# bcgsc/ntSynt

Hardware: AMD Instinct MI355X
Metric: minimizer-sketch Gbases/s (sketch with common Bloom filter, inputs resident in HBM) (higher is better)
Workload: dtype u64

## Files before the change

include/ntsynt_hip.h:

```cpp
#ifndef NTSYNT_HIP_H
#define NTSYNT_HIP_H

#include <stdint.h>

#ifdef __cplusplus
extern "C" {
#endif

#define NTS_OK 0
#define NTS_EINVAL (-22)
#define NTS_ENOMEM (-12)
#define NTS_EHIP (-5)
#define NTS_ERANGE (-34)
#define NTS_EFORMAT (-74)
#define NTS_ECOMM (-70)

typedef struct nts_ctx nts_ctx;
typedef struct nts_genome nts_genome;
typedef struct nts_bf nts_bf;
typedef struct nts_mx nts_mx;
typedef struct nts_hset nts_hset;
typedef struct nts_hcount nts_hcount;
typedef struct nts_comm nts_comm;

// ... 44 lines not shown
#define NTS_SYNTH_NRUN 4u
typedef struct
{
  uint64_t dst, len, src;
  uint32_t flags, reserved;
} nts_synth_piece;
int nts_genome_synth_plan(nts_ctx* ctx, uint32_t n_rec, const uint64_t* rec_len, uint32_t n_pieces, const nts_synth_piece* pieces,
                          uint64_t seed_ancestor, uint64_t seed_genome, double substitution_rate, nts_genome** out);
#define NTS_SYNTH_TANDEM 8u
typedef struct
{
  uint32_t sine_cell_log2, sine_len, sine_prob_256, sine_families;
  uint32_t line_cell_log2, line_len, line_min_len, line_prob_256, line_families;
  uint32_t div_min_1024, div_max_1024;
  uint32_t sat_unit, sat_div_1024;
} nts_synth_repeats;
int nts_genome_synth_plan_ex(nts_ctx* ctx, uint32_t n_rec, const uint64_t* rec_len, uint32_t n_pieces, const nts_synth_piece* pieces,
                             uint64_t seed_ancestor, uint64_t seed_genome, double substitution_rate, const nts_synth_repeats* rep,
                             nts_genome** out);
int nts_genome_download(nts_ctx* ctx, const nts_genome* g, uint64_t offset, uint64_t len, uint8_t* ascii);
uint64_t nts_genome_bases(const nts_genome* g);
int nts_genome_valid_kmers(nts_ctx* ctx, const nts_genome* g, uint32_t k, uint64_t* n_valid);

int nts_bf_create(nts_ctx* ctx, uint64_t bytes, nts_bf** out);
void nts_bf_free(nts_ctx* ctx, nts_bf* bf);
uint64_t nts_bf_bytes(const nts_bf* bf);
void* nts_bf_device_ptr(nts_bf* bf);
int nts_bf_clear(nts_ctx* ctx, nts_bf* bf);
int nts_bf_insert_and(nts_ctx* ctx, nts_bf* acc, const nts_genome* g, uint32_t k);
int nts_bf_insert(nts_ctx* ctx, nts_bf* bf, const nts_genome* g, uint32_t k);
int nts_bf_build_mode(nts_ctx* ctx, int mode);
int nts_bf_cascade(nts_ctx* ctx, const nts_bf* prev, nts_bf* next, const nts_genome* g, uint32_t k);
int nts_bf_insert_repeats(nts_ctx* ctx, nts_bf* genome_bf, nts_bf* repeat_bf, const nts_genome* g, uint32_t k);
int nts_bf_and(nts_ctx* ctx, nts_bf* acc, const nts_bf* other);
int nts_bf_popcount(nts_ctx* ctx, const nts_bf* bf, uint64_t* bits_set);
int nts_bf_download(nts_ctx* ctx, const nts_bf* bf, uint8_t* host, uint64_t bytes);
int nts_bf_upload(nts_ctx* ctx, nts_bf* bf, const uint8_t* host, uint64_t bytes);
int nts_bf_save(nts_ctx* ctx, const nts_bf* bf, const char* path, const void* header, uint64_t header_bytes, uint32_t n_threads);
int nts_bench_random_probe(nts_ctx* ctx, const nts_bf* bf, uint64_t n_probes, uint32_t repeats, double* avg_ms, uint64_t* hits);
int nts_bench_valu(nts_ctx* ctx, int kind, uint32_t waves_per_simd, uint32_t iters, double* wall_ms, double* cycles_per_instr,
                   double* instr_per_wave);
int nts_mod_indices(nts_ctx* ctx, uint64_t bits, int form, const uint64_t* h, uint64_t n, uint64_t* out);
int nts_bf_wrap(nts_ctx* ctx, void* device_ptr, uint64_t bytes, nts_bf** out);
int nts_and_raw(nts_ctx* ctx, void* acc_dev, const void* other_dev, uint64_t bytes);

int nts_comm_unique_id(uint8_t* id128);
int nts_comm_init(nts_ctx* ctx, const uint8_t* id128, int world, int rank, nts_comm** out);
int nts_comm_wrap(nts_ctx* ctx, void* rccl_comm, nts_comm** out);
void nts_comm_destroy(nts_comm* comm);
int nts_comm_world(const nts_comm* comm);
int nts_comm_rank(const nts_comm* comm);
void* nts_comm_handle(const nts_comm* comm);
const char* nts_comm_library(void);
int nts_bf_create_sharded(nts_ctx* ctx, uint64_t bytes, int world, nts_bf** out);
int nts_bf_fill_ones(nts_ctx* ctx, nts_bf* bf);
int nts_bf_allreduce_and(nts_ctx* ctx, nts_bf* bf, nts_comm* comm);
int nts_bf_allreduce_groups(nts_ctx* ctx, nts_bf* bf, nts_comm* comm, const int32_t* group_of, uint32_t n_groups);
int nts_comm_last_sparse(const nts_ctx* ctx);
int nts_comm_last_exchange2(const nts_ctx* ctx, uint64_t* packed_bytes, uint64_t* unpacked_bytes, uint64_t* sent_bytes);
int nts_bf_allreduce_parts(nts_ctx* ctx, nts_bf* const* bfs, uint32_t n_local, nts_comm* comm, uint32_t n_slots, const int32_t* slot_group,
                           uint32_t n_groups);
int nts_mx_allgather(nts_ctx* ctx, nts_comm* comm, uint32_t n_local, const nts_mx* const* local, const uint32_t* local_ids,
                     uint32_t n_total, nts_mx** out);
int nts_mx_allgather_ex(nts_ctx* ctx, nts_comm* comm, uint32_t n_local, const nts_mx* const* local, const uint32_t* local_ids,
                        uint32_t n_total, uint32_t slots_per_rank, nts_mx** out);

int nts_sketch(nts_ctx* ctx,
               const nts_genome* g,
               uint32_t k,
               uint32_t w,
               const nts_bf* filter_or_null,
               const nts_interval* mask,
               uint64_t n_mask,
               nts_mx** out);

int nts_sketch_ex(nts_ctx* ctx, const nts_genome* g, uint32_t k, uint32_t w, const nts_bf* filter, const nts_bf* filter_out,
                  const nts_interval* mask, uint64_t n_mask, nts_mx** out);
int nts_sketch_mode(nts_ctx* ctx, int mode, uint32_t prune_c);
int nts_sketch_summary(nts_ctx* ctx, int mode, uint32_t* last_shift);
int nts_sketch_select(nts_ctx* ctx, int impl);
int nts_sketch_tiers(nts_ctx* ctx, int mode, double x0, int half_steps, uint64_t* last_probes, uint64_t* last_rounds, uint32_t* last_tiers);
int nts_sketch_stats(nts_ctx* ctx, uint64_t* candidates, uint64_t* uncovered_ranges, uint64_t* uncovered_kmers, uint32_t* prune_c_used);
int nts_path_stats(nts_ctx* ctx, uint64_t* sketch_many_listed, uint64_t* bf_direct_indices, uint32_t* bf_list_fallback);
int nts_bf_level_stats(nts_ctx* ctx, uint32_t* sparse_level, uint64_t* accepted_kmers);
uint64_t nts_mx_count(const nts_mx* mx);
void nts_mx_free(nts_ctx* ctx, nts_mx* mx);
int nts_mx_download(nts_ctx* ctx, const nts_mx* mx, uint64_t* h1, uint32_t* rec, uint64_t* pos);
int nts_mx_device_ptrs(const nts_mx* mx, void** h1, void** rec, void** pos);
int nts_mx_export(nts_ctx* ctx, const nts_mx* mx, void* h1_dev, void* rec_dev, void* pos_dev);
int nts_mx_export_async(nts_ctx* ctx, const nts_mx* mx, void* h1_dev, void* rec_dev, void* pos_dev);
int nts_mx_kmers(nts_ctx* ctx, const nts_genome* g, const nts_mx* mx, uint32_t k, uint8_t* host);
int nts_mx_split(nts_ctx* ctx, const nts_mx* mx, uint32_t n_parts, const uint32_t* rec_base, nts_mx** out);
int nts_mx_concat(nts_ctx* ctx, uint32_t n_parts, const nts_mx* const* parts, const uint32_t* rec_offset, nts_mx** out);
int nts_mx_screen(nts_ctx* ctx, const nts_genome* g, const nts_mx* mx, uint32_t k, const nts_bf* filter_out, nts_mx** out);
int nts_mx_upload(nts_ctx* ctx,
                  const uint64_t* h1,
                  const uint32_t* rec,
                  const uint64_t* pos,
                  uint64_t n,
                  nts_mx** out);

int nts_hash_all(nts_ctx* ctx, const nts_genome* g, uint32_t k, uint64_t** h0, uint64_t* n_out);

int nts_minhash(nts_ctx* ctx, const nts_genome* g, uint32_t k, uint32_t s, uint64_t* out, uint32_t* n_out);

int nts_minhash_intervals(nts_ctx* ctx, const nts_genome* g, uint32_t k, uint32_t s, const nts_interval* iv, uint64_t n_iv, uint64_t* out,
                          uint32_t* n_out, uint64_t* n_kmers);
int nts_minhash_intervals_stats(nts_ctx* ctx, uint32_t* passes, uint32_t* chunks, uint64_t* sweeps);
int nts_minhash_pairs(nts_ctx* ctx, uint32_t s, const uint64_t* sk, const uint32_t* n_sk, uint64_t n_sketches, const uint64_t* pair_a,
                      const uint64_t* pair_b, uint64_t n_pairs, uint32_t* shared, uint32_t* usize);

int nts_bf_count_intervals(nts_ctx* ctx, const nts_genome* g, uint32_t k, const nts_bf* bf, const nts_interval* iv, uint64_t n_iv,
                           uint64_t* n_kmers, uint64_t* n_hits);
int nts_genome_valid_bases(nts_ctx* ctx, const nts_genome* g, const nts_interval* iv, uint64_t n_iv, uint64_t* n_valid);

typedef struct
{
  uint64_t h0;
  uint32_t iv;
  uint32_t off;
} nts_sample;
typedef struct
{
  uint32_t list_a, iv_a, list_b, iv_b;
  uint32_t anchors, fwd, rev;
  uint32_t min_off_a, max_off_a, min_off_b, max_off_b;
} nts_iv_link;
int nts_bf_sample_intervals(nts_ctx* ctx, const nts_genome* g, uint32_t k, const nts_bf* bf, uint64_t rate, const nts_interval* iv,
                            uint64_t n_iv, uint64_t* n_sampled, nts_sample** out, uint64_t* n_out);
int nts_iv_links(nts_ctx* ctx, uint32_t n_lists, const nts_sample* const* lists, const uint64_t* n, uint32_t min_anchors, nts_iv_link** out,
                 uint64_t* n_out);

int nts_hset_build(nts_ctx* ctx, const uint64_t* h, uint64_t n, nts_hset** out);
void nts_hset_free(nts_ctx* ctx, nts_hset* set);
int nts_hset_contains(nts_ctx* ctx, const nts_hset* set, const uint64_t* h, uint64_t n, uint8_t* out);
int nts_hset_sample_intervals(nts_ctx* ctx, const nts_genome* g, uint32_t k, const nts_hset* set, uint64_t rate, const nts_interval* iv,
                              uint64_t n_iv, uint64_t* n_sampled, nts_sample** out, uint64_t* n_out);

int nts_hcount_create(nts_ctx* ctx, const nts_hset* set, nts_hcount** out);
int nts_hcount_clear(nts_ctx* ctx, nts_hcount* cnt);
void nts_hcount_free(nts_ctx* ctx, nts_hcount* cnt);
int nts_hcount_add(nts_ctx* ctx, const nts_hset* set, nts_hcount* cnt, const uint64_t* h, uint64_t n);
int nts_hcount_read(nts_ctx* ctx, const nts_hset* set, const nts_hcount* cnt, const uint64_t* h, uint64_t n, uint32_t* out);
int nts_hset_count_intervals(nts_ctx* ctx, const nts_genome* g, uint32_t k, const nts_hset* set, nts_hcount* cnt, uint64_t rate,
                             const nts_interval* iv, uint64_t n_iv, uint64_t* n_hits);

typedef struct
{
  uint32_t list_q, iv_q, rec_t;
  uint32_t hits, fwd, rev;
  uint32_t min_off_q, max_off_q, first_t, last_t;
} nts_iv_site;
int nts_hset_sample_intervals_capped(nts_ctx* ctx, const nts_genome* g, uint32_t k, const nts_hset* set, const nts_hcount* cnt, uint32_t cap,
                                     uint64_t rate, const nts_interval* iv, uint64_t n_iv, uint64_t* n_sampled, nts_sample** out, uint64_t* n_out);
int nts_iv_sites(nts_ctx* ctx, uint32_t n_lists, const nts_sample* const* lists, const uint64_t* n, const nts_sample* target, uint64_t n_target,
                 uint32_t step, uint32_t min_hits, nts_iv_site** out, uint64_t* n_out);

typedef struct
{
  uint32_t recurring, period, period_hits, first_off, last_off;
} nts_iv_period;
int nts_sample_intervals(nts_ctx* ctx, const nts_genome* g, uint32_t k, uint64_t rate, const nts_interval* iv, uint64_t n_iv, uint64_t* n_sampled,
                         nts_sample** out, uint64_t* n_out);
int nts_iv_periods(nts_ctx* ctx, const nts_sample* recs, uint64_t n, uint64_t n_iv, nts_iv_period* out);

typedef struct
// ... 137 lines not shown
```

ntsynt_amd/_lib.py:

```python
import ctypes
import os
import subprocess

_HERE = os.path.dirname(os.path.abspath(__file__))
LIB_PATH = os.path.join(_HERE, "libntsynt_hip.so")
EXP_LIB_PATH = os.path.join(_HERE, "libntsynt_hip_exp.so")

c_u8p = ctypes.POINTER(ctypes.c_uint8)
c_u32p = ctypes.POINTER(ctypes.c_uint32)
c_i64p = ctypes.POINTER(ctypes.c_int64)
c_u64p = ctypes.POINTER(ctypes.c_uint64)
c_vp = ctypes.c_void_p
u32, u64 = ctypes.c_uint32, ctypes.c_uint64


class Interval(ctypes.Structure):
    _fields_ = [("rec", u32), ("start", u64), ("end", u64)]


class Sample(ctypes.Structure):
    _fields_ = [("h0", u64), ("iv", u32), ("off", u32)]


class IvLink(ctypes.Structure):
# ... 45 lines not shown
class Blocks(ctypes.Structure):
    _fields_ = [("n_blocks", u64), ("first_vid", c_u32p), ("last_vid", c_u32p), ("n_mx", c_u32p), ("rec", c_u32p),
                ("first_pos", c_u64p), ("last_pos", c_u64p), ("ori", c_u8p), ("stats_paths", u64), ("stats_unoriented", u64),
                ("stats_indel_cuts", u64), ("stats_small", u64)]


SYMBOLS = [
    ("nts_init", ctypes.c_int, [ctypes.c_int, ctypes.POINTER(c_vp)]),
    ("nts_destroy", None, [c_vp]),
    ("nts_last_error", ctypes.c_char_p, [c_vp]),
    ("nts_sync", ctypes.c_int, [c_vp]),
    ("nts_stream", c_vp, [c_vp]),
    ("nts_profile", ctypes.c_int, [c_vp, ctypes.c_int]),
    ("nts_timing", ctypes.c_int, [c_vp, ctypes.c_char_p, ctypes.POINTER(ctypes.c_double), c_u64p]),
    ("nts_mem_stats", ctypes.c_int, [c_vp, c_u64p, c_u64p, c_u64p, c_u64p]),
    ("nts_mem_reset_peak", None, []),
    ("nts_bf_size_bytes", ctypes.c_int, [u64, ctypes.c_double, c_u64p, c_u64p]),
    ("nts_bf_size_bytes_ex", ctypes.c_int, [u64, ctypes.c_double, ctypes.c_int, c_u64p, c_u64p]),
    ("nts_genome_upload", ctypes.c_int, [c_vp, c_vp, u64, c_u64p, c_u64p, u32, ctypes.POINTER(c_vp)]),
    ("nts_genome_synth", ctypes.c_int, [c_vp, u64, u32, u64, u64, ctypes.c_double, ctypes.POINTER(c_vp)]),
    ("nts_genome_synth_plan", ctypes.c_int, [c_vp, u32, c_vp, u32, c_vp, u64, u64, ctypes.c_double, ctypes.POINTER(c_vp)]),
    ("nts_genome_synth_plan_ex", ctypes.c_int, [c_vp, u32, c_vp, u32, c_vp, u64, u64, ctypes.c_double, c_vp, ctypes.POINTER(c_vp)]),
    ("nts_genome_download", ctypes.c_int, [c_vp, c_vp, u64, u64, c_vp]),
    ("nts_genome_concat", ctypes.c_int, [c_vp, u32, c_vp, ctypes.POINTER(c_vp)]),
    ("nts_genome_slice", ctypes.c_int, [c_vp, c_vp, u32, u32, ctypes.POINTER(c_vp)]),
    ("nts_genome_free", None, [c_vp, c_vp]),
    ("nts_genome_bases", u64, [c_vp]),
    ("nts_genome_valid_kmers", ctypes.c_int, [c_vp, c_vp, u32, c_u64p]),
    ("nts_bf_create", ctypes.c_int, [c_vp, u64, ctypes.POINTER(c_vp)]),
    ("nts_bf_free", None, [c_vp, c_vp]),
    ("nts_bf_bytes", u64, [c_vp]),
    ("nts_bf_device_ptr", c_vp, [c_vp]),
    ("nts_bf_clear", ctypes.c_int, [c_vp, c_vp]),
    ("nts_bf_insert", ctypes.c_int, [c_vp, c_vp, c_vp, u32]),
    ("nts_bf_insert_and", ctypes.c_int, [c_vp, c_vp, c_vp, u32]),
    ("nts_bf_build_mode", ctypes.c_int, [c_vp, ctypes.c_int]),
    ("nts_bf_cascade", ctypes.c_int, [c_vp, c_vp, c_vp, c_vp, u32]),
    ("nts_bf_insert_repeats", ctypes.c_int, [c_vp, c_vp, c_vp, c_vp, u32]),
    ("nts_bf_and", ctypes.c_int, [c_vp, c_vp, c_vp]),
    ("nts_bf_popcount", ctypes.c_int, [c_vp, c_vp, c_u64p]),
    ("nts_bf_download", ctypes.c_int, [c_vp, c_vp, c_vp, u64]),
    ("nts_bf_upload", ctypes.c_int, [c_vp, c_vp, c_vp, u64]),
    ("nts_bf_save", ctypes.c_int, [c_vp, c_vp, ctypes.c_char_p, c_vp, u64, u32]),
    ("nts_bench_random_probe", ctypes.c_int, [c_vp, c_vp, u64, u32, ctypes.POINTER(ctypes.c_double), c_u64p]),
    ("nts_bench_valu", ctypes.c_int, [c_vp, ctypes.c_int, u32, u32, ctypes.POINTER(ctypes.c_double),
                                      ctypes.POINTER(ctypes.c_double), ctypes.POINTER(ctypes.c_double)]),
    ("nts_mod_indices", ctypes.c_int, [c_vp, u64, ctypes.c_int, c_vp, u64, c_vp]),
    ("nts_bf_wrap", ctypes.c_int, [c_vp, c_vp, u64, ctypes.POINTER(c_vp)]),
    ("nts_and_raw", ctypes.c_int, [c_vp, c_vp, c_vp, u64]),
    ("nts_comm_unique_id", ctypes.c_int, [c_vp]),
    ("nts_comm_init", ctypes.c_int, [c_vp, c_vp, ctypes.c_int, ctypes.c_int, ctypes.POINTER(c_vp)]),
    ("nts_comm_wrap", ctypes.c_int, [c_vp, c_vp, ctypes.POINTER(c_vp)]),
    ("nts_comm_destroy", None, [c_vp]),
    ("nts_comm_world", ctypes.c_int, [c_vp]),
    ("nts_comm_rank", ctypes.c_int, [c_vp]),
    ("nts_comm_handle", c_vp, [c_vp]),
    ("nts_comm_library", ctypes.c_char_p, []),
    ("nts_bf_create_sharded", ctypes.c_int, [c_vp, u64, ctypes.c_int, ctypes.POINTER(c_vp)]),
    ("nts_bf_fill_ones", ctypes.c_int, [c_vp, c_vp]),
    ("nts_bf_allreduce_and", ctypes.c_int, [c_vp, c_vp, c_vp]),
    ("nts_bf_allreduce_groups", ctypes.c_int, [c_vp, c_vp, c_vp, ctypes.POINTER(ctypes.c_int32), u32]),
    ("nts_comm_last_sparse", ctypes.c_int, [c_vp]),
    ("nts_comm_last_exchange2", ctypes.c_int, [c_vp, c_vp, c_vp, c_vp]),
    ("nts_mx_allgather", ctypes.c_int, [c_vp, c_vp, u32, ctypes.POINTER(c_vp), c_u32p, u32, ctypes.POINTER(c_vp)]),
    ("nts_alloc_stats", ctypes.c_int, [c_vp, c_vp]),
    ("nts_mem_trim", ctypes.c_uint64, []),
    ("nts_mem_cache_stats", ctypes.c_int, [c_vp, c_vp]),
    ("nts_mem_reserve", ctypes.c_int, [ctypes.c_int, ctypes.c_uint64, c_vp]),
    ("nts_mem_events", ctypes.c_int, [c_vp]),
    ("nts_mx_allgather_ex", ctypes.c_int, [c_vp, c_vp, u32, ctypes.POINTER(c_vp), c_u32p, u32, u32, ctypes.POINTER(c_vp)]),
    ("nts_bf_allreduce_parts", ctypes.c_int, [c_vp, ctypes.POINTER(c_vp), u32, c_vp, u32, ctypes.POINTER(ctypes.c_int32), u32]),
    ("nts_mx_export", ctypes.c_int, [c_vp, c_vp, c_vp, c_vp, c_vp]),
    ("nts_mx_export_async", ctypes.c_int, [c_vp, c_vp, c_vp, c_vp, c_vp]),
    ("nts_sketch", ctypes.c_int, [c_vp, c_vp, u32, u32, c_vp, ctypes.POINTER(Interval), u64,
                                  ctypes.POINTER(c_vp)]),
    ("nts_sketch_ex", ctypes.c_int, [c_vp, c_vp, u32, u32, c_vp, c_vp, ctypes.POINTER(Interval), u64,
                                     ctypes.POINTER(c_vp)]),
    ("nts_sketch_mode", ctypes.c_int, [c_vp, ctypes.c_int, u32]),
    ("nts_sketch_summary", ctypes.c_int, [c_vp, ctypes.c_int, c_u32p]),
    ("nts_sketch_select", ctypes.c_int, [c_vp, ctypes.c_int]),
    ("nts_sketch_tiers", ctypes.c_int, [c_vp, ctypes.c_int, ctypes.c_double, ctypes.c_int, ctypes.c_void_p, ctypes.c_void_p, ctypes.c_void_p]),
    ("nts_sketch_stats", ctypes.c_int, [c_vp, c_u64p, c_u64p, c_u64p, c_u32p]),
    ("nts_path_stats", ctypes.c_int, [c_vp, c_u64p, c_u64p, c_u32p]),
    ("nts_bf_level_stats", ctypes.c_int, [c_vp, c_u32p, c_u64p]),
    ("nts_mx_count", u64, [c_vp]),
    ("nts_mx_free", None, [c_vp, c_vp]),
    ("nts_mx_download", ctypes.c_int, [c_vp, c_vp, c_vp, c_vp, c_vp]),
    ("nts_mx_device_ptrs", ctypes.c_int, [c_vp, ctypes.POINTER(c_vp), ctypes.POINTER(c_vp),
                                          ctypes.POINTER(c_vp)]),
    ("nts_mx_split", ctypes.c_int, [c_vp, c_vp, u32, c_u32p, ctypes.POINTER(c_vp)]),
    ("nts_mx_concat", ctypes.c_int, [c_vp, u32, ctypes.POINTER(c_vp), c_u32p, ctypes.POINTER(c_vp)]),
    ("nts_mx_screen", ctypes.c_int, [c_vp, c_vp, c_vp, u32, c_vp, ctypes.POINTER(c_vp)]),
    ("nts_mx_upload", ctypes.c_int, [c_vp, c_vp, c_vp, c_vp, u64, ctypes.POINTER(c_vp)]),
    ("nts_hash_all", ctypes.c_int, [c_vp, c_vp, u32, ctypes.POINTER(c_u64p), c_u64p]),
    ("nts_minhash", ctypes.c_int, [c_vp, c_vp, u32, u32, c_u64p, c_u32p]),
    ("nts_minhash_intervals", ctypes.c_int, [c_vp, c_vp, u32, u32, ctypes.POINTER(Interval), u64, c_vp, c_vp, c_vp]),
    ("nts_minhash_intervals_stats", ctypes.c_int, [c_vp, c_u32p, c_u32p, c_u64p]),
    ("nts_bf_count_intervals", ctypes.c_int, [c_vp, c_vp, u32, c_vp, ctypes.POINTER(Interval), u64, c_vp, c_vp]),
    ("nts_bf_sample_intervals", ctypes.c_int, [c_vp, c_vp, u32, c_vp, u64, ctypes.POINTER(Interval), u64, c_vp, ctypes.POINTER(c_vp), c_u64p]),
    ("nts_iv_links", ctypes.c_int, [c_vp, u32, ctypes.POINTER(c_vp), c_u64p, u32, ctypes.POINTER(c_vp), c_u64p]),
    ("nts_hset_build", ctypes.c_int, [c_vp, c_vp, u64, ctypes.POINTER(c_vp)]),
    ("nts_hset_free", None, [c_vp, c_vp]),
    ("nts_hset_contains", ctypes.c_int, [c_vp, c_vp, c_vp, u64, c_vp]),
    ("nts_hset_sample_intervals", ctypes.c_int, [c_vp, c_vp, u32, c_vp, u64, ctypes.POINTER(Interval), u64, c_vp, ctypes.POINTER(c_vp), c_u64p]),
    ("nts_hcount_create", ctypes.c_int, [c_vp, c_vp, ctypes.POINTER(c_vp)]),
    ("nts_hcount_clear", ctypes.c_int, [c_vp, c_vp]),
    ("nts_hcount_free", None, [c_vp, c_vp]),
    ("nts_hcount_add", ctypes.c_int, [c_vp, c_vp, c_vp, c_vp, u64]),
    ("nts_hcount_read", ctypes.c_int, [c_vp, c_vp, c_vp, c_vp, u64, c_vp]),
    ("nts_hset_count_intervals", ctypes.c_int, [c_vp, c_vp, u32, c_vp, c_vp, u64, ctypes.POINTER(Interval), u64, c_vp]),
    ("nts_hset_sample_intervals_capped", ctypes.c_int, [c_vp, c_vp, u32, c_vp, c_vp, u32, u64, ctypes.POINTER(Interval), u64, c_vp, ctypes.POINTER(c_vp),
                                                        c_u64p]),
    ("nts_iv_sites", ctypes.c_int, [c_vp, u32, ctypes.POINTER(c_vp), c_u64p, c_vp, u64, u32, u32, ctypes.POINTER(c_vp), c_u64p]),
    ("nts_sample_intervals", ctypes.c_int, [c_vp, c_vp, u32, u64, ctypes.POINTER(Interval), u64, c_vp, ctypes.POINTER(c_vp), c_u64p]),
    ("nts_iv_periods", ctypes.c_int, [c_vp, c_vp, u64, u64, c_vp]),
    ("nts_genome_valid_bases", ctypes.c_int, [c_vp, c_vp, ctypes.POINTER(Interval), u64, c_vp]),
    ("nts_minhash_pairs", ctypes.c_int, [c_vp, u32, c_vp, c_vp, u64, c_vp, c_vp, u64, c_vp, c_vp]),
    ("nts_graph_build", ctypes.c_int, [c_vp, u32, ctypes.POINTER(MxList), ctypes.POINTER(Graph)]),
    ("nts_graph_budget", ctypes.c_int, [c_vp, u64]),
    ("nts_graph_last_plan", ctypes.c_int, [c_vp, c_u32p, c_u32p, c_u64p, c_u32p]),
    ("nts_graph_plan_slices", ctypes.c_int, [c_vp, u32, u64, u64, c_vp, c_vp]),
    ("nts_engine_create", ctypes.c_int, [c_vp, u32, u32, ctypes.POINTER(c_vp)]),
    ("nts_engine_free", None, [c_vp, c_vp]),
    ("nts_engine_size", ctypes.c_int, [c_vp, c_u64p, c_u64p]),
    ("nts_engine_add", ctypes.c_int, [c_vp, c_vp, ctypes.POINTER(c_vp), ctypes.POINTER(Spans), c_u64p, c_u64p]),
    ("nts_engine_bubbles", ctypes.c_int, [c_vp, c_vp, ctypes.POINTER(Bubbles)]),
    ("nts_bubbles_free", None, [ctypes.POINTER(Bubbles)]),
    ("nts_engine_apply", ctypes.c_int, [c_vp, c_vp, c_vp, u64, c_vp, u64, u32]),
    ("nts_engine_filter", ctypes.c_int, [c_vp, c_vp, u32, ctypes.c_int, c_u64p]),
    ("nts_engine_erode", ctypes.c_int, [c_vp, c_vp, u32, c_u64p]),
    ("nts_engine_blocks", ctypes.c_int, [c_vp, c_vp, ctypes.c_int64, ctypes.c_double, u32, ctypes.POINTER(Blocks)]),
    ("nts_blocks_free", None, [ctypes.POINTER(Blocks)]),
    ("nts_engine_paths", ctypes.c_int, [c_vp, c_u64p, c_u64p]),
    ("nts_engine_read", ctypes.c_int, [c_vp, c_vp, ctypes.c_char_p, c_vp, u64]),
    ("nts_bubble_rule", ctypes.c_int, [u64, c_vp, u64, c_vp, c_vp, c_vp, c_vp, u32, c_vp, c_vp, c_u64p]),
    ("nts_blocks_merge", ctypes.c_int, [u32, u64, ctypes.c_int64, ctypes.c_int64, ctypes.c_int64, c_vp, c_vp, c_vp, c_vp, c_vp, c_vp,
                                        c_u64p, c_u64p]),
    ("nts_blocks_text", ctypes.c_int, [u32, u64, ctypes.c_int64, ctypes.c_int64, c_vp, ctypes.c_char_p, u64, c_vp, c_vp, c_vp, c_vp,
                                       c_vp, c_vp, c_vp, ctypes.POINTER(c_vp), c_u64p]),
    ("nts_walk_chains", ctypes.c_int, [u64, u64, c_vp, c_vp, ctypes.POINTER(c_u64p), ctypes.POINTER(c_u32p), c_u64p]),
    ("nts_walk_paths", ctypes.c_int, [u64, u64, c_vp, c_vp, c_vp, c_vp, ctypes.POINTER(c_u64p), ctypes.POINTER(c_i64p), c_u64p]),
    ("nts_edge_degrees", ctypes.c_int, [u64, u64, c_vp, c_vp, c_vp, c_vp]),
    ("nts_to_i64", ctypes.c_int, [c_vp, u32, u64, c_vp]),
    ("nts_path_scan", ctypes.c_int, [u32, u64, c_vp, c_vp, u64, c_vp, c_vp, ctypes.c_int64, c_vp, c_vp, c_vp]),
    ("nts_graph_free", None, [ctypes.POINTER(Graph)]),
    ("nts_fasta_read", ctypes.c_int, [ctypes.c_char_p, ctypes.POINTER(Fasta)]),
    ("nts_fasta_free", None, [ctypes.POINTER(Fasta)]),
    ("nts_read_indexlr_tsv", ctypes.c_int, [ctypes.c_char_p, ctypes.POINTER(MxTsv)]),
    ("nts_mx_tsv_free", None, [ctypes.POINTER(MxTsv)]),
    ("nts_genome_from_fasta", ctypes.c_int, [c_vp, ctypes.c_char_p, ctypes.POINTER(c_vp), ctypes.POINTER(Fasta)]),
    ("nts_ingest_trim", ctypes.c_int, [c_vp]),
    ("nts_bf_build_trim", ctypes.c_int, [c_vp]),
    ("nts_mx_kmers", ctypes.c_int, [c_vp, c_vp, c_vp, u32, c_vp]),
    ("nts_write_indexlr_tsv_kmers", ctypes.c_int, [ctypes.c_char_p, ctypes.POINTER(Fasta), c_vp, c_vp, c_vp, u64, u32, c_vp]),
    ("nts_write_indexlr_tsv", ctypes.c_int, [ctypes.c_char_p, ctypes.POINTER(Fasta), c_vp, c_vp, c_vp, u64, u32, ctypes.c_int]),
    ("nts_free", None, [c_vp]),
]


def build(force=False):
    args = ["make", "-s", "-C", os.path.join(_HERE, "csrc")]
    if force:
        args.append("-B")
    subprocess.run(args, check=True)
    return LIB_PATH

# ... 24 lines not shown
```

ntsynt_amd/csrc/nts_internal.h:

```cpp
#pragma once
#include <hip/hip_runtime.h>

#include <execinfo.h>
#include <fcntl.h>
#include <sys/mman.h>
#include <sys/stat.h>
#include <unistd.h>
#include <mutex>
#include <thread>

#include <algorithm>
#include <cmath>
#include <cstdint>
#include <cstdlib>
#include <cstring>
#include <atomic>
#include <chrono>
#include <map>
#include <set>
#include <string>
#include <tuple>
#include <vector>

#include <rocprim/rocprim.hpp>
// ... 339 lines not shown
  AllocClock clk;
  return ::hipFree(p);
}
}
using nts_mem::dev_free;
using nts_mem::dev_malloc;
using nts_mem::dev_malloc_flags;

inline std::atomic<int> g_live_contexts{0};
namespace nts_chain {
inline std::mutex mu;
inline hipEvent_t ev[32] = {};
inline bool live[32] = {};
}

namespace {

constexpr uint64_t PAD = 256;
constexpr int HASH_THREADS = 256;
constexpr int HASH_PER_THREAD = 32;
constexpr int WIN_THREADS = 512;
constexpr uint32_t WIN_TILE = 4096;
constexpr uint32_t WIN_CHUNK = 16;
constexpr uint32_t WIN_MAX_W = 12000;
constexpr uint32_t MAIL_WORDS = 32768;

std::string g_init_error;

struct Timing
{
  double ms = 0;
  uint64_t launches = 0;
};

}

struct nts_ctx
{
  int device = 0;
  bool counted = false;
  hipStream_t stream = nullptr;
  hipStream_t copy_stream = nullptr;
  uint64_t* mail = nullptr;
  uint64_t* d_mail = nullptr;
  uint64_t mail_seq = 0;
  uint8_t* stage = nullptr;
  size_t stage_bytes = 0;
  std::string err;
  int profiling = 0;
  std::map<std::string, Timing> timings;
  std::vector<std::pair<std::string, std::pair<hipEvent_t, hipEvent_t>>> pending;
  std::map<uint32_t, uint64_t*> init_tabs;
  std::vector<hipEvent_t> spare_events;
  std::map<std::string, std::pair<void*, size_t>> ws;
  std::vector<std::pair<void*, uint64_t>> mx_pool;
  size_t win_lds_set = 0;
  bool bin_lds_set = false;
  uint32_t n_cus = 0;
  bool sel_ctl_clean = false;
  int bf_build_mode = 0;
  int sketch_mode = 0;
  uint32_t prune_c = 0;
  uint32_t last_c = 0;
  uint64_t last_candidates = 0, last_gaps = 0, last_gap_kmers = 0;
  uint64_t last_many_listed = 0;
  uint64_t last_bf_direct = 0;
  size_t win_fused_lds_set = 0;
  uint32_t last_comm_sparse = 0;
  uint64_t last_x2_packed_bytes = 0, last_x2_unpacked_bytes = 0, last_x2_sent_bytes = 0;
  uint32_t last_bf_fallback = 0;
  uint32_t last_bf_sparse_level = 0;
  uint64_t last_bf_sparse_accepted = 0;
  int fold_mode = 0;
  bool acc4_lds_set = false;
  bool acc4r_lds_set = false;
  struct IoLane
  {
    hipStream_t stream = nullptr;
    uint8_t* stage[2] = { nullptr, nullptr };
  };
  std::vector<IoLane> io_up, io_down;
  double dense_seg_per_window = 3.0;
  double fused_seg_per_window = 2.5;
  bool elim_needs_full_cap = false;
  int select_impl = 0;
  int summary_mode = 0;
  uint32_t last_summary = 0;
  uint64_t comm_piece = 0;
  int comm_sparse_mode = 0;
  uint64_t comm_sparse_below = 0;
  unsigned io_threads = 8;
  int gap_tiers_off = 0;
  int tier_mode = 0;
  double tier_x0 = 0;
  uint32_t tier_half = 0;
  uint64_t last_tier_probes = 0, last_tier_rounds = 0, last_tiers = 0;
  uint64_t graph_budget = 0;
  uint32_t last_graph_v_slices = 0, last_graph_e_slices = 0, last_graph_oversize = 0;
  uint64_t last_graph_peak = 0;
  uint64_t graph_live0 = 0;
  uint32_t last_mhi_passes = 0, last_mhi_chunks = 0;
  uint64_t last_mhi_sweeps = 0;
};

struct nts_genome
{
  uint64_t n = 0;
  uint32_t n_rec = 0;
  uint8_t* d_code = nullptr;
  mutable uint32_t* d_pack = nullptr;
  std::vector<uint64_t> rec_off, rec_len;
  uint64_t total_bases = 0;
  std::vector<uint64_t> part_bases;
  std::vector<uint64_t> st_a, st_b;
  uint64_t* d_rec_off = nullptr;
  mutable std::map<uint32_t, struct GenomeTables*> tables;
};

struct nts_bf
{
  uint64_t bytes = 0;
  uint64_t alloc_bytes = 0;
  uint32_t* d_words = nullptr;
  bool owned = true;
  mutable int64_t popcnt = -1;
  uint64_t version = 0;
  mutable uint32_t* d_summary = nullptr;
  mutable uint64_t summary_words = 0;
  mutable uint32_t summary_shift = 0;
  mutable uint64_t summary_version = ~0ULL;
  mutable double summary_density = 1.0;
  mutable uint32_t* d_fold = nullptr;
  mutable std::mutex mu;
};

struct nts_hset
{
  uint64_t* d_slots = nullptr;
  uint64_t n_slots = 0;
  uint32_t shift = 0;
  uint64_t n_in = 0;
  bool has_max = false;
  int device = 0;
};

struct nts_hcount
{
  uint32_t* d_cnt = nullptr;
  const nts_hset* set = nullptr;
  uint64_t n_slots = 0;
  uint64_t offered = 0;
  int device = 0;
};

struct nts_mx
{
  uint64_t n = 0;
  uint64_t cap_bytes = 0;
  uint64_t* d_h1 = nullptr;
  uint32_t* d_rec = nullptr;
  uint64_t* d_pos = nullptr;
};

namespace {

inline std::atomic<uint64_t> g_refused_launches{0};
// ... 314 lines not shown
```

ntsynt_amd/csrc/nts_pruned.inc:

```
constexpr uint32_t SEL_CAP = 2048;
constexpr uint32_t SEL_PER_LANE = 64;
constexpr uint32_t SEL_TILE = HASH_THREADS * SEL_PER_LANE;
constexpr uint32_t SPARSE_THREADS = 256;
constexpr uint32_t SPARSE_ITEMS = 2;
constexpr uint32_t SPARSE_BLOCK = SPARSE_THREADS * SPARSE_ITEMS;
constexpr uint32_t CC_TILES = 8;

struct SelParams
{
  const uint8_t* code;
  const uint32_t* pack;
  const uint64_t* run_pos;
  const uint64_t* run_vstart;
  uint32_t n_runs;
  uint64_t n_valid;
  HashParams hp;
  const uint32_t* bf;
  FastMod fm;
  uint64_t tau;
  uint32_t flush_at;
  uint64_t* seg_j;
  uint64_t* seg_key;
  uint64_t seg_cap;
  unsigned long long* seg_count;
  uint64_t* tile_off;
  uint32_t* tile_cnt;
  uint8_t* tile_ordered;
  uint32_t w_elim;
};




template <uint32_t SEL_SLOTS>
__global__ __launch_bounds__(HASH_THREADS) void k_hash_select(SelParams P)
{
  struct Lds
  {
    uint64_t tab[36];
    uint64_t ch[(SEL_SLOTS + 1) * HASH_THREADS];
    uint16_t ci[SEL_SLOTS * HASH_THREADS];
    uint32_t ctl[4];
    unsigned long long base;
  };
  __shared__ Lds lds;
  uint64_t* const s_tab = lds.tab;
  uint64_t* const s_ch = lds.ch;
  uint16_t* const s_ci = lds.ci;
  uint32_t* const s_ctl = lds.ctl;
  unsigned long long& s_base = lds.base;
  const uint32_t tid = threadIdx.x;
  if (tid < 16) {
    s_tab[tid] = P.hp.roll_f[tid];
    s_tab[16 + tid] = P.hp.roll_r[tid];
  }
  if (tid < 4) s_tab[32 + tid] = P.hp.seed[tid];
  if (tid == 0) s_ctl[0] = s_ctl[1] = 0;
  const uint32_t k = P.hp.k;
  const uint64_t tile = blockIdx.x;
  const uint64_t J0 = tile * SEL_TILE;
  const uint32_t tile_len = (uint32_t)min((uint64_t)SEL_TILE, P.n_valid - J0);
  uint32_t lo = 0, hi = P.n_runs;
  while (hi - lo > 1) {
    const uint32_t mid = lo + ((hi - lo) >> 1);
    if (P.run_vstart[mid] <= J0)
      lo = mid;
    else
      hi = mid;
  }
  const uint64_t v0 = P.run_vstart[lo], v1 = P.run_vstart[lo + 1];
  const bool single = (J0 + tile_len <= v1) && (k <= FAST_K_MAX);
  const bool hi_only = (uint32_t)P.tau == 0xFFFFFFFFu;
  const uint32_t first = SEL_PER_LANE * tid;
  const uint32_t n_mine = first < tile_len ? min(SEL_PER_LANE, tile_len - first) : 0u;
  const uint64_t tau = P.tau;
  const uint64_t P0 = single ? P.run_pos[lo] + (J0 - v0) : 0;
  auto base_abs = [&](uint64_t p) -> uint32_t { return (P.pack[p >> 4] >> (2u * ((uint32_t)p & 15u))) & 3u; };
  __syncthreads();

  auto roll_pass = [&](uint32_t r_lo, uint32_t r_hi) {
    if (n_mine == 0 || first >= r_hi || first + n_mine <= r_lo) return;
    auto consider = [&](uint64_t h, uint32_t idx) {
      if (h <= tau && idx >= r_lo && idx < r_hi) {
        const uint32_t slot = atomicAdd(&s_ctl[0], 1u);
        if (slot < SEL_CAP) {
          s_ch[slot] = h;
          s_ci[slot] = (uint16_t)idx;
        }
      }
    };
    if (single) {
      uint64_t s = P0 + first;
      uint64_t f = 0, r = 0;
      hash_init(P.hp, [&](uint32_t i) { return base_abs(s + i); }, f, r);
      for (uint32_t u = 0; u < n_mine; ++u) {
        consider(f + r, first + u);
        const uint32_t cout = base_abs(s), cin = base_abs(s + k);
        f = srol1(f) ^ s_tab[cin * 4 + cout];
        r = sror1(r ^ s_tab[16 + cin * 4 + cout]);
        ++s;
      }
    } else {
      uint64_t j = J0 + first;
      const uint64_t j_end = j + n_mine;
      uint32_t rl = 0, rh = P.n_runs;
      while (rh - rl > 1) {
        const uint32_t mid = rl + ((rh - rl) >> 1);
        if (P.run_vstart[mid] <= j)
          rl = mid;
        else
          rh = mid;
// ... 471 lines not shown
    run = run_next;
    single = J0 + len <= v1 ? 1u : 0u;
    P0 = sload64(P.run_pos, run_next) + (J0 - sload64(P.run_vstart, run_next));
  };
  uint32_t run_end = P.n_runs;
  auto position_of = [&](uint64_t j, uint32_t run_lo) -> uint64_t {
    uint32_t rl = run_lo, rh = run_end;
    while (rh - rl > 1) {
      const uint32_t mid = rl + ((rh - rl) >> 1);
      if (P.run_vstart[mid] <= j)
        rl = mid;
      else
        rh = mid;
    }
    return P.run_pos[rl] + (j - P.run_vstart[rl]);
  };
  auto stage_dma = [&](uint64_t t_P0, bool real, uint32_t buf) {
    const uint64_t w0 = real ? ((t_P0 >> 4) & ~3ULL) : 0ULL;
    const uint32_t lds = stage_lds + buf * (HIW_STAGE_WORDS * 4u);
    const uint32_t* ga = P.pack + w0 + 4u * lane;
    asm volatile("s_mov_b32 m0, %1\n\ts_nop 0\n\tglobal_load_lds_dwordx4 %0, off" ::"v"(ga), "s"(lds) : "memory");
    if (lane < 4) {
      const uint32_t* gb = ga + 256;
      asm volatile("s_mov_b32 m0, %1\n\ts_nop 0\n\tglobal_load_lds_dwordx4 %0, off" ::"v"(gb), "s"(lds + 1024u) : "memory");
    }
  };
  auto full_hash = [&](const uint32_t* words, uint32_t sh) -> uint64_t {
    const uint32_t w0 = words[0], w1 = words[1], w2 = words[2];
    const uint32_t b_lo = __builtin_amdgcn_alignbit(w1, w0, sh), b_hi = __builtin_amdgcn_alignbit(w2, w1, sh);
    uint64_t f = 0, r = 0;
#pragma unroll
    for (uint32_t c = 0; c < HI_K_MAX / 4; ++c) {
      if (c < nch) {
        const ulonglong2 e = s_T[c * 256u + (((c < 4 ? b_lo : b_hi) >> (8u * (c & 3u))) & 255u)];
        f ^= e.x;
        r ^= e.y;
      }
    }
    return f + r;
  };

  uint64_t pd_h[HIW_PER];
  uint32_t pd_i[HIW_PER], pd_w[HIW_PER], pd_b[HIW_PER];
  uint32_t pd_m = 0;
  uint64_t pd_tile = ~0ULL, pd_J0 = 0;
  uint32_t pd_single = 0;
#pragma unroll
  for (uint32_t i = 0; i < HIW_PER; ++i) {
    pd_h[i] = 0;
    pd_i[i] = 0;
    pd_w[i] = 0;
    pd_b[i] = 0;
  }
  auto issue_probes = [&]() {
    if (HAS_BF) {
      const uint32_t* wp[HIW_PER];
#pragma unroll
      for (uint32_t i = 0; i < HIW_PER; ++i) {
        const uint64_t bidx = P.fm(pd_h[i]);
        pd_b[i] = (uint32_t)bidx & 31u;
        wp[i] = P.bf + (((pd_m >> i) & 1u) ? (bidx >> 5) : 0ULL);
      }
#pragma unroll
      for (uint32_t i = 0; i < HIW_PER; ++i)
        asm volatile("s_mov_b32 m0, %1\n\ts_nop 0\n\tglobal_load_lds_dword %0, off" ::"v"(wp[i]), "s"(probe_lds + i * 256u) : "memory");
    }
  };
  auto wait_stage = [&]() {
    if (HAS_BF && HIW_PER == 4)
      asm volatile("s_waitcnt vmcnt(6)" ::: "memory");
    else if (HAS_BF)
      asm volatile("s_waitcnt vmcnt(4)" ::: "memory");
    else
      asm volatile("s_waitcnt vmcnt(2)" ::: "memory");
  };
  auto wait_probes = [&]() {
    if (HAS_BF) {
      asm volatile("s_waitcnt vmcnt(0)" ::: "memory");
#pragma unroll
      for (uint32_t i = 0; i < HIW_PER; ++i) pd_w[i] = s_probe[wv][i][lane];
    }
  };
  uint32_t wave_run = 0;
  auto finish_pending = [&]() {
    if (pd_tile == ~0ULL) return;
    uint32_t okm = pd_m;
    if (HAS_BF) {
#pragma unroll
      for (uint32_t i = 0; i < HIW_PER; ++i)
        if (!((pd_w[i] >> pd_b[i]) & 1u)) okm &= ~(1u << i);
    }
    uint32_t rank = 0, accepted = 0;
#pragma unroll
    for (uint32_t i = 0; i < HIW_PER; ++i) {
      const unsigned long long bm = __ballot((okm >> i) & 1u);
      rank += (uint32_t)__popcll(bm & below);
      accepted += (uint32_t)__popcll(bm);
    }
    if (P.w_elim && pd_single && accepted > 2u && accepted + 2u * ELIM_REACH <= HIW_LIST) {
      uint32_t* const s_e = &s_probe[wv][0][0];
      if (lane < 2u * ELIM_REACH) s_e[lane < ELIM_REACH ? lane : accepted + lane] = 0xFFFFFFFFu;
      uint32_t n = 0;
#pragma unroll
      for (uint32_t i = 0; i < HIW_PER; ++i) {
        if ((okm >> i) & 1u) {
          s_e[ELIM_REACH + rank + n] = ((uint32_t)(pd_h[i] >> key16_shift) << 16) | pd_i[i];
          ++n;
        }
      }
      __builtin_amdgcn_fence(__ATOMIC_RELEASE, "wavefront");
      __builtin_amdgcn_wave_barrier();
      __builtin_amdgcn_fence(__ATOMIC_ACQUIRE, "wavefront");
      unsigned long long lost[HIW_PER];
#pragma unroll
      for (uint32_t ps = 0; ps < HIW_PER; ++ps) {
        lost[ps] = 0ULL;
        if (64u * ps < accepted) {
          const uint32_t* const me = s_e + ELIM_REACH + min(64u * ps + lane, accepted - 1u);
          const uint32_t floor16 = *me & 0xFFFF0000u;
          uint32_t wl = 0xFFFFFFFFu, wr = 0xFFFFFFFFu;
#pragma unroll
          for (int s1 = (int)ELIM_REACH; s1 >= 1; --s1) {
            const uint32_t L = me[-s1], R = me[s1];
            wl = L < floor16 ? L : wl;
            wr = R < floor16 ? R : wr;
          }
          const bool both = (wl & wr) != 0xFFFFFFFFu && wl != 0xFFFFFFFFu && wr != 0xFFFFFFFFu;
          lost[ps] = __ballot(64u * ps + lane < accepted && both && ((wr & 0xFFFFu) - (wl & 0xFFFFu) <= P.w_elim));
        }
      }
      uint32_t dead = 0;
#pragma unroll
      for (uint32_t i = 0; i < HIW_PER; ++i) {
        const uint32_t e = rank + (uint32_t)__popc(okm & ((1u << i) - 1u));
        unsigned long long m = lost[0];
#pragma unroll
        for (uint32_t ps = 1; ps < HIW_PER; ++ps) m = (e >> 6) == ps ? lost[ps] : m;
        if (((okm >> i) & 1u) && ((m >> (e & 63u)) & 1ULL)) dead |= 1u << i;
      }
      __builtin_amdgcn_wave_barrier();
      okm &= ~dead;
      rank = 0;
      accepted = 0;
#pragma unroll
      for (uint32_t i = 0; i < HIW_PER; ++i) {
        const unsigned long long bm = __ballot((okm >> i) & 1u);
        rank += (uint32_t)__popcll(bm & below);
        accepted += (uint32_t)__popcll(bm);
      }
    }
    const uint64_t list_at = tile_first * HIW_LIST + wave_run;
    const uint64_t dst = list_at + rank;
    wave_run += accepted;
    if (lane == 0) {
      P.tile_off[pd_tile] = list_at;
      P.tile_cnt[pd_tile] = accepted;
      P.tile_ordered[pd_tile] = 1;
    }
    uint32_t n = 0;
#pragma unroll
    for (uint32_t i = 0; i < HIW_PER; ++i) {
      if ((okm >> i) & 1u) {
        P.seg_j[dst + n] = pd_J0 + pd_i[i];
        P.seg_key[dst + n] = pd_h[i];
        ++n;
      }
// ... 78 lines not shown
        const unsigned long long hm = __ballot(hit);
        if (lane == o) {
          pen0 = (uint32_t)hm;
          pen1 = (uint32_t)(hm >> 32);
        }
      }
    }
    const uint32_t cnt = (uint32_t)__popc(pen0) + (uint32_t)__popc(pen1);
    uint32_t C = 0;
    const uint32_t off = wave_excl_scan_small(cnt, below, &C);
    auto build_list = [&](uint32_t rb) {
      if (off + cnt > rb && off < rb + HIW_LIST) {
        uint32_t pos = off - rb;
        uint32_t a = pen0, b = pen1;
        while (a) {
          const uint32_t s1 = (uint32_t)__builtin_ctz(a);
          a &= a - 1u;
          if (pos < HIW_LIST) s_list[pos] = (uint16_t)(first + s1);
          ++pos;
        }
        while (b) {
          const uint32_t s1 = (uint32_t)__builtin_ctz(b);
          b &= b - 1u;
          if (pos < HIW_LIST) s_list[pos] = (uint16_t)(first + 32u + s1);
          ++pos;
        }
      }
      __builtin_amdgcn_fence(__ATOMIC_RELEASE, "wavefront");
      __builtin_amdgcn_wave_barrier();
    };
    auto hash_round = [&](uint32_t rb, uint64_t (&h)[HIW_PER], uint32_t (&ix)[HIW_PER]) -> uint32_t {
      const uint32_t n = min(HIW_LIST, C - rb);
      const uint32_t per = (n + 63u) >> 6;
      const uint32_t e0 = lane * per;
      uint32_t m = 0;
#pragma unroll
      for (uint32_t i = 0; i < HIW_PER; ++i) {
        h[i] = 0;
        ix[i] = 0;
        if (i < per && e0 + i < n) {
          const uint32_t idx = s_list[e0 + i];
          ix[i] = idx;
          if (g.single) {
            const uint64_t p = g.P0 + idx;
            h[i] = full_hash(st + (uint32_t)((p >> 4) - w0), 2u * ((uint32_t)p & 15u));
          } else {
            const uint64_t p = position_of(g.J0 + idx, g.run);
            h[i] = full_hash(P.pack + (p >> 4), 2u * ((uint32_t)p & 15u));
          }
          if (h[i] <= P.tau) m |= 1u << i;
        }
      }
      __builtin_amdgcn_wave_barrier();
      return m;
    };
    if (C <= HIW_LIST) {
      build_list(0);
      uint64_t nh[HIW_PER];
      uint32_t ni[HIW_PER];
      const uint32_t nm = hash_round(0, nh, ni);
      wait_probes();
      finish_pending();
#pragma unroll
      for (uint32_t i = 0; i < HIW_PER; ++i) {
        pd_h[i] = nh[i];
        pd_i[i] = ni[i];
      }
      pd_m = nm;
      pd_tile = tile;
      pd_J0 = g.J0;
      pd_single = g.single ? 1u : 0u;
    } else {
      wait_probes();
      finish_pending();
      const uint32_t seg = (uint32_t)(tile % N_SEG);
      uint32_t listed_ok = 0, accepted = 0;
      unsigned long long base = 0;
      bool fits = true;
      for (int sweep = 0; sweep < 2 && fits; ++sweep) {
        if (sweep == 1) {
          if (lane == 0) base = listed_ok ? atomicAdd(&P.seg_count[seg], (unsigned long long)listed_ok) : 0ULL;
          base = __shfl(base, 0, 64);
          fits = base + listed_ok <= P.seg_cap;
          if (listed_ok == 0 || !fits) break;
        }
        uint64_t dst = n_tiles * HIW_LIST + (uint64_t)seg * P.seg_cap + base;
        for (uint32_t rb = 0; rb < C; rb += HIW_LIST) {
          build_list(rb);
          uint64_t h[HIW_PER];
          uint32_t ix[HIW_PER];
          uint32_t okm = hash_round(rb, h, ix);
          if (HAS_BF && sweep == 1) {
#pragma unroll
            for (uint32_t i = 0; i < HIW_PER; ++i)
              if (((okm >> i) & 1u) && !bf_test(P.bf, P.fm(h[i]))) okm &= ~(1u << i);
          }
          uint32_t rank = 0, acc = 0;
#pragma unroll
          for (uint32_t i = 0; i < HIW_PER; ++i) {
            const unsigned long long bm = __ballot((okm >> i) & 1u);
            rank += (uint32_t)__popcll(bm & below);
            acc += (uint32_t)__popcll(bm);
          }
          if (sweep == 0) {
            listed_ok += acc;
          } else {
            uint32_t n = 0;
#pragma unroll
            for (uint32_t i = 0; i < HIW_PER; ++i) {
              if ((okm >> i) & 1u) {
                P.seg_j[dst + rank + n] = g.J0 + ix[i];
                P.seg_key[dst + rank + n] = h[i];
                ++n;
              }
            }
            dst += acc;
            accepted += acc;
          }
        }
      }
      if (lane == 0) {
        P.tile_off[tile] = fits ? n_tiles * HIW_LIST + (uint64_t)seg * P.seg_cap + base : ~0ULL;
        P.tile_cnt[tile] = fits ? accepted : 0u;
        P.tile_ordered[tile] = 1;
      }
    }
  }
  issue_probes();
  wait_probes();
  finish_pending();
}

__global__ __launch_bounds__(256) void k_cand_compact(const uint64_t* __restrict__ seg_j, const uint64_t* __restrict__ seg_key,
                                                      uint64_t seg_cap, const uint64_t* __restrict__ tile_off,
                                                      const uint32_t* __restrict__ tile_cnt, const uint8_t* __restrict__ tile_ordered,
                                                      const uint64_t* __restrict__ out_off, uint64_t n_tiles, uint64_t* __restrict__ pj,
                                                      uint64_t* __restrict__ pk, uint64_t cap, unsigned long long* __restrict__ overflow,
                                                      bool absolute)
{
  __shared__ uint64_t s_k[SEL_CAP];
  __shared__ uint64_t s_k2[SEL_CAP];
  __shared__ uint16_t s_i[SEL_CAP];
  __shared__ uint16_t s_i2[SEL_CAP];
  __shared__ uint32_t s_hist[256];
  __shared__ uint32_t s_base[257];
  __shared__ uint32_t s_w[8];
  __shared__ uint32_t s_n;
  __shared__ uint32_t s_todo[CC_TILES];
  __shared__ uint32_t s_ntodo;
  if (threadIdx.x == 0) s_ntodo = 0;
  __syncthreads();
  {
    const uint64_t t = (uint64_t)blockIdx.x * CC_TILES + (threadIdx.x >> 5);
    const uint32_t l32 = threadIdx.x & 31u;
    if (t < n_tiles) {
      const uint32_t n = tile_cnt[t];
      const bool fits = absolute ? tile_off[t] != ~0ULL : tile_off[t] + n <= seg_cap;
      if (n != 0 && !fits && l32 == 0) *overflow = 1ULL;
      if (n != 0 && fits) {
        if (tile_ordered[t]) {
          const uint64_t src = absolute ? tile_off[t] : (t % N_SEG) * seg_cap + tile_off[t];
          const uint64_t dst = out_off[t];
          for (uint32_t e = l32; e < n; e += 32) {
            if (dst + e < cap) {
              pj[dst + e] = seg_j[src + e];
              pk[dst + e] = seg_key[src + e];
            }
          }
        } else if (l32 == 0) {
          s_todo[atomicAdd(&s_ntodo, 1u)] = (uint32_t)(threadIdx.x >> 5);
        }
      }
    }
  }
  __syncthreads();
  const uint32_t n_todo = s_ntodo;
  for (uint32_t td = 0; td < n_todo; ++td) {
  const uint64_t tile = (uint64_t)blockIdx.x * CC_TILES + s_todo[td];
  const uint32_t n = tile_cnt[tile];
  const uint64_t src = (tile % N_SEG) * seg_cap + tile_off[tile];
  uint64_t dst = out_off[tile];
  const uint64_t J0 = tile * SEL_TILE;
  const uint32_t n_ranges = n <= SEL_CAP ? 1u : SEL_TILE / 2048u;
  for (uint32_t r = 0; r < n_ranges; ++r) {
    const uint64_t lo = n_ranges == 1 ? J0 : J0 + 2048ull * r;
    const uint64_t hi = n_ranges == 1 ? J0 + SEL_TILE : lo + 2048ull;
    __syncthreads();
    if (threadIdx.x == 0) s_n = 0;
    s_hist[threadIdx.x] = 0;
    __syncthreads();
    for (uint32_t i = threadIdx.x; i < n; i += 256) {
      const uint64_t j = seg_j[src + i];
      if (j >= lo && j < hi) {
        const uint32_t slot = atomicAdd(&s_n, 1u);
        if (slot < SEL_CAP) {
          const uint32_t idx = (uint32_t)(j - J0);
          s_i[slot] = (uint16_t)idx;
          s_k[slot] = seg_key[src + i];
          atomicAdd(&s_hist[idx >> 6], 1u);
        }
      }
    }
    __syncthreads();
    const uint32_t c = min(s_n, SEL_CAP);
    uint32_t tot = 0;
    const uint32_t mine = s_hist[threadIdx.x];
    const uint32_t base = block_excl_scan_256(mine, s_w, &tot);
    s_base[threadIdx.x] = base;
    if (threadIdx.x == 255) s_base[256] = base + mine;
    s_hist[threadIdx.x] = 0;
    __syncthreads();
    for (uint32_t e = threadIdx.x; e < c; e += 256) {
      const uint32_t b = s_i[e] >> 6;
// ... 11 lines not shown
        while (y > b0 && s_i2[y - 1] > vi) {
          s_i2[y] = s_i2[y - 1];
          s_k2[y] = s_k2[y - 1];
          --y;
        }
        s_i2[y] = vi;
        s_k2[y] = vk;
      }
    }
    __syncthreads();
    for (uint32_t e = threadIdx.x; e < c; e += 256) {
      if (dst + e < cap) {
        pj[dst + e] = J0 + s_i2[e];
        pk[dst + e] = s_k2[e];
      }
    }
    dst += c;
  }
  }
}

constexpr uint32_t CCS_TILES = 16;

__global__ __launch_bounds__(256) void k_cand_compact_slots(const uint64_t* __restrict__ seg_j, const uint64_t* __restrict__ seg_key,
                                                            const uint64_t* __restrict__ tile_off, const uint32_t* __restrict__ tile_cnt,
                                                            const uint64_t* __restrict__ out_off, uint64_t n_tiles, uint64_t* __restrict__ pj,
                                                            uint64_t* __restrict__ pk, uint64_t cap, unsigned long long* __restrict__ overflow)
{
  const uint64_t t = (uint64_t)blockIdx.x * CCS_TILES + (threadIdx.x >> 4);
  const uint32_t l16 = threadIdx.x & 15u;
  if (t >= n_tiles) return;
  const uint32_t n = tile_cnt[t];
  const uint64_t src = tile_off[t];
  const uint64_t dst = out_off[t];
  if (n == 0) return;
  if (src == ~0ULL) {
    if (l16 == 0) *overflow = 1ULL;
    return;
  }
  for (uint32_t e = l16; e < n; e += 16) {
    if (dst + e < cap) {
      pj[dst + e] = seg_j[src + e];
      pk[dst + e] = seg_key[src + e];
    }
  }
}

struct SparseParams
{
  const uint64_t* pj;
  const uint64_t* pk;
  const uint64_t* m_scan_last;
  const uint32_t* m_cnt_last;
  uint64_t m_max;
  const uint64_t* rec_vstart;
  const uint64_t* rec_nv;
  uint64_t n_valid;
  uint32_t n_rec;
  uint32_t w;
  uint64_t* stage_j;
  uint64_t* stage_k;
  uint64_t* blk_cnt;
  uint64_t* gap_lo;
  uint64_t* gap_hi;
  unsigned long long* gap_count;
  uint64_t gap_cap;
  const unsigned long long* overflow;
  uint32_t rec_holes = 0;
  uint32_t no_gaps = 0;
};

__device__ __forceinline__ void push_gap(const SparseParams& P, uint64_t lo, uint64_t hi)
{
  const unsigned long long s = atomicAdd(P.gap_count, 1ULL);
  if (s < P.gap_cap) {
    P.gap_lo[s] = lo;
    P.gap_hi[s] = hi;
  }
}

constexpr uint32_t SPARSE_HALO = 64;
constexpr uint32_t SPARSE_REC_LDS = 2048;

__global__ __launch_bounds__(SPARSE_THREADS) void k_sparse_win(SparseParams P)
{
  __shared__ uint32_t s_wcnt[SPARSE_THREADS / 64];
  __shared__ ulonglong2 s_c[SPARSE_BLOCK + 2 * SPARSE_HALO];
  __shared__ uint64_t s_rv[SPARSE_REC_LDS];
  const uint64_t m = *P.overflow ? 0 : min(*P.m_scan_last + (uint64_t)*P.m_cnt_last, P.m_max);
  if (!*P.overflow && !P.no_gaps)
    for (uint64_t r = (uint64_t)blockIdx.x * SPARSE_THREADS + threadIdx.x; r < P.n_rec; r += (uint64_t)gridDim.x * SPARSE_THREADS) {
      const uint64_t rs = P.rec_vstart[r], nv = P.rec_nv[r];
      if (nv < P.w) continue;
      uint64_t lo = 0, hi = m;
      while (lo < hi) {
        const uint64_t mid = lo + ((hi - lo) >> 1);
        if (P.pj[mid] < rs)
          lo = mid + 1;
        else
          hi = mid;
      }
      if (lo >= m || P.pj[lo] >= rs + nv) push_gap(P, rs, rs + nv - 1);
    }
  if ((uint64_t)blockIdx.x * SPARSE_BLOCK >= m) {
    if (threadIdx.x == 0) P.blk_cnt[blockIdx.x] = 0;
    return;
  }
  const uint64_t blk0 = (uint64_t)blockIdx.x * SPARSE_BLOCK;
  const uint64_t lds_lo = blk0 >= SPARSE_HALO ? blk0 - SPARSE_HALO : 0;
  const uint64_t lds_hi = min(m, blk0 + SPARSE_BLOCK + SPARSE_HALO);
  for (uint64_t q = lds_lo + threadIdx.x; q < lds_hi; q += SPARSE_THREADS) {
    s_c[q - lds_lo] = make_ulonglong2(P.pj[q], P.pk[q]);
  }
  const bool recs_in_lds = P.n_rec <= SPARSE_REC_LDS && !P.rec_holes;
  if (recs_in_lds)
    for (uint32_t q = threadIdx.x; q < P.n_rec; q += SPARSE_THREADS) s_rv[q] = P.rec_vstart[q];
  __syncthreads();
  auto cand_j = [&](uint64_t q) -> uint64_t { return (q >= lds_lo && q < lds_hi) ? s_c[q - lds_lo].x : P.pj[q]; };
  auto cand_k = [&](uint64_t q) -> uint64_t { return (q >= lds_lo && q < lds_hi) ? s_c[q - lds_lo].y : P.pk[q]; };
  const uint32_t lane = threadIdx.x & 63u, wv = threadIdx.x >> 6;
  uint32_t winners_so_far = 0;
  for (uint32_t item = 0; item < SPARSE_ITEMS; ++item) {
  const uint64_t i = blk0 + (uint64_t)item * SPARSE_THREADS + threadIdx.x;
  bool win = false;
  uint64_t j = 0, key = 0;
  if (i < m) {
    j = cand_j(i);
    key = cand_k(i);
    uint32_t lo = 0, hi = P.n_rec;
    if (recs_in_lds) {
      while (hi - lo > 1) {
        const uint32_t mid = lo + ((hi - lo) >> 1);
        if (s_rv[mid] <= j)
          lo = mid;
        else
          hi = mid;
      }
    } else {
      while (hi - lo > 1) {
        const uint32_t mid = lo + ((hi - lo) >> 1);
        if (P.rec_vstart[mid] <= j)
          lo = mid;
        else
          hi = mid;
      }
    }
    uint64_t rs, re;
    if (recs_in_lds) {
      rs = s_rv[lo];
      re = lo + 1 < P.n_rec ? s_rv[lo + 1] : P.n_valid;
    } else {
      rs = P.rec_vstart[lo];
      re = rs + P.rec_nv[lo];
    }
    const uint64_t w = P.w;
    if (re - rs >= w) {
      const uint64_t a_lim = (j - rs >= w - 1) ? j - (w - 1) : rs;
      const uint64_t b_lim = (re - 1 - j >= w - 1) ? j + (w - 1) : re - 1;
      uint64_t a_min = a_lim, b_max = b_lim;
      const uint32_t li = (uint32_t)(i - lds_lo), n_st = (uint32_t)(lds_hi - lds_lo);
      bool redo_left = lds_lo > 0, redo_right = lds_hi < m;
      {
        constexpr uint32_t STOPPED = 0x80000000u;
        uint32_t ql = li, qr = li;
        for (;;) {
          const bool gl = ql - 1u < STOPPED - 1u;
          const bool gr = qr + 1u < n_st;
          if (!(gl | gr)) break;
          const uint32_t il = ql - (gl ? 1u : 0u), ir = qr + (gr ? 1u : 0u);
          const ulonglong2 L = s_c[min(il, n_st - 1u)], R = s_c[min(ir, n_st - 1u)];
          ql = (gl & ((L.x < a_lim) | (L.y < key))) ? (il | STOPPED) : il;
          qr = (gr & ((R.x > b_lim) | (R.y <= key))) ? (ir | STOPPED) : ir;
        }
        if (ql & STOPPED) {
          const uint64_t x = s_c[ql & ~STOPPED].x;
          if (x >= a_lim) a_min = x + 1;
        }
        if (qr & STOPPED) {
          const uint64_t x = s_c[qr & ~STOPPED].x;
          if (x <= b_lim) b_max = x - 1;
        }
        redo_left = redo_left & (ql == 0u);
        redo_right = redo_right & (qr + 1u == n_st);
      }
      if (redo_left) {
        a_min = a_lim;
        for (uint64_t q = i; q-- > 0;) {
          const uint64_t jq = cand_j(q);
          if (jq < a_lim) break;
          if (cand_k(q) < key) {
            a_min = jq + 1;
            break;
          }
        }
      }
      if (redo_right) {
        b_max = b_lim;
        for (uint64_t q = i + 1; q < m; ++q) {
          const uint64_t jq = cand_j(q);
          if (jq > b_lim) break;
          if (cand_k(q) <= key) {
            b_max = jq - 1;
            break;
          }
        }
      }
      bool have_next = false;
      uint64_t j_next = 0;
      if (i + 1 < m) {
        j_next = s_c[li + 1].x;
        have_next = j_next < re;
      }
      win = b_max - a_min + 1 >= w;
      const uint64_t nxt = have_next ? j_next : re;
      if (!P.no_gaps) {
        if (nxt - j - 1 >= w) push_gap(P, j + 1, nxt - 1);
        const bool first_in_rec = (i == 0) || (s_c[li - 1].x < rs);
        if (first_in_rec && j - rs >= w) push_gap(P, rs, j - 1);
      }
    }
  }
  const unsigned long long bal = __ballot(win);
  if (item) __syncthreads();
  if (lane == 0) s_wcnt[wv] = (uint32_t)__popcll(bal);
  __syncthreads();
  uint32_t base = 0, total = 0;
  for (uint32_t q = 0; q < SPARSE_THREADS / 64; ++q) {
    const uint32_t c = s_wcnt[q];
    if (q < wv) base += c;
    total += c;
  }
  if (win) {
    const uint32_t r = winners_so_far + base + (uint32_t)__popcll(bal & ((1ULL << lane) - 1ULL));
    P.stage_j[blk0 + r] = j;
    P.stage_k[blk0 + r] = key;
  }
  winners_so_far += total;
  }
  if (threadIdx.x == 0) P.blk_cnt[blockIdx.x] = winners_so_far;
}

__global__ __launch_bounds__(256) void k_gather_winners(const uint64_t* __restrict__ stage_j, const uint64_t* __restrict__ stage_k,
                                                       const uint64_t* __restrict__ blk_cnt, const uint64_t* __restrict__ blk_scan,
                                                       uint64_t* __restrict__ out_j, uint64_t* __restrict__ out_k)
{
  const uint64_t b = blockIdx.x;
  const uint64_t n = blk_cnt[b], dst = blk_scan[b], src = b * SPARSE_BLOCK;
  for (uint64_t i = threadIdx.x; i < n; i += 256) {
    out_j[dst + i] = stage_j[src + i];
    out_k[dst + i] = stage_k[src + i];
  }
}

__global__ __launch_bounds__(256) void k_merge_lists(const uint64_t* __restrict__ a_j, const uint64_t* __restrict__ a_k, uint64_t na,
                                                    const uint64_t* __restrict__ b_j, const uint64_t* __restrict__ b_k, uint64_t nb,
                                                    uint64_t* __restrict__ out_j, uint64_t* __restrict__ out_k)
{
  const uint64_t t = (uint64_t)blockIdx.x * blockDim.x + threadIdx.x;
  if (t >= na + nb) return;
  const bool from_a = t < na;
  const uint64_t self = from_a ? t : t - na;
  const uint64_t key = from_a ? a_j[self] : b_j[self];
  const uint64_t* other = from_a ? b_j : a_j;
  uint64_t lo = 0, hi = from_a ? nb : na;
  while (lo < hi) {
    const uint64_t mid = lo + ((hi - lo) >> 1);
    if (other[mid] < key)
      lo = mid + 1;
    else
      hi = mid;
  }
  out_j[self + lo] = key;
  out_k[self + lo] = from_a ? a_k[self] : b_k[self];
}

constexpr uint32_t GAP_TILE_CAP = 128;
constexpr uint32_t GAP_TILES_MAX = 4096;
constexpr uint32_t GAP_LIST_CAP = 65536;
constexpr uint32_t GAP_COLLECT_THREADS = 1024;

__global__ __launch_bounds__(GAP_COLLECT_THREADS) void k_gap_collect(const uint32_t* __restrict__ tile_cnt, uint32_t n_tiles,
                                                                     const uint64_t* __restrict__ tile_j,
                                                                     const uint64_t* __restrict__ tile_key, uint64_t n_sparse,
                                                                     uint64_t* __restrict__ out_j, uint64_t* __restrict__ out_key,
                                                                     uint64_t* __restrict__ ctl)
{
  static_assert(GAP_TILES_MAX == 4 * GAP_COLLECT_THREADS, "four tiles per lane");
  __shared__ uint32_t s_off[GAP_TILES_MAX + 1];
  __shared__ uint32_t s_wave[GAP_COLLECT_THREADS / 64];
  __shared__ uint32_t s_bad;
  const uint32_t tid = threadIdx.x, lane = tid & 63u, wv = tid >> 6;
  if (tid == 0) s_bad = 0;
  uint32_t c[4], sum = 0;
  bool bad = false;
#pragma unroll
  for (uint32_t q = 0; q < 4; ++q) {
    const uint32_t t = 4u * tid + q;
    c[q] = t < n_tiles ? tile_cnt[t] : 0u;
    bad |= c[q] > GAP_TILE_CAP;
    c[q] = min(c[q], GAP_TILE_CAP);
    sum += c[q];
  }
  uint32_t inc = sum;
#pragma unroll
  for (int d = 1; d < 64; d <<= 1) {
    const uint32_t up = __shfl_up(inc, d, 64);
    if ((int)lane >= d) inc += up;
  }
  if (lane == 63) s_wave[wv] = inc;
  __syncthreads();
  if (bad) s_bad = 1;
  uint32_t before = inc - sum;
  for (uint32_t x = 0; x < wv; ++x) before += s_wave[x];
#pragma unroll
  for (uint32_t q = 0; q < 4; ++q) {
    s_off[4u * tid + q] = before;
    before += c[q];
  }
  if (tid == GAP_COLLECT_THREADS - 1) s_off[GAP_TILES_MAX] = before;
  __syncthreads();
  const uint32_t n = s_off[GAP_TILES_MAX];
  if (s_bad || n > GAP_LIST_CAP) {
// ... 648 lines not shown
```

ntsynt_amd/csrc/ntsynt_hip.hip:

```cpp
#include "nts_internal.h"

namespace {


__global__ __launch_bounds__(256) void k_encode(uint8_t* __restrict__ buf, uint64_t n)
{
  const uint64_t i = ((uint64_t)blockIdx.x * blockDim.x + threadIdx.x) * 16;
  if (i >= n) return;
  if (i + 16 <= n) {
    uint4 v = *reinterpret_cast<const uint4*>(buf + i);
    uint32_t wds[4] = { v.x, v.y, v.z, v.w };
#pragma unroll
    for (int q = 0; q < 4; ++q) {
      uint32_t out = 0;
#pragma unroll
      for (int b = 0; b < 4; ++b) {
        uint32_t c = (wds[q] >> (8 * b)) & 0xFFu;
        c &= 0xDFu;
        uint32_t code = (c == 'A') ? 0u : (c == 'C') ? 1u : (c == 'G') ? 2u : (c == 'T' || c == 'U') ? 3u : 4u;
        out |= code << (8 * b);
      }
      wds[q] = out;
    }
    *reinterpret_cast<uint4*>(buf + i) = make_uint4(wds[0], wds[1], wds[2], wds[3]);
// ... 394 lines not shown
        const uint32_t cout = base_at(s2), cin = base_at(s2 + k);
        f2 = srol1(f2) ^ s_tab[cin * 4 + cout];
        r2 = sror1(r2 ^ s_tab[16 + cin * 4 + cout]);
        ++s2;
      }
    }
    return;
  }
  __syncthreads();
  if (tid == 0) tile_any[blockIdx.x] = 1u;
  uint64_t j = J0 + 32ull * tid;
  if (j >= n_valid) return;
  const uint64_t j_end = min(j + (uint64_t)HASH_PER_THREAD, n_valid);
  lo = 0;
  hi = n_runs;
  while (hi - lo > 1) {
    const uint32_t mid = lo + ((hi - lo) >> 1);
    if (run_vstart[mid] <= j)
      lo = mid;
    else
      hi = mid;
  }
  uint32_t ri = lo;
  while (j < j_end) {
    const uint64_t rv0 = run_vstart[ri], rv1 = run_vstart[ri + 1];
    const uint64_t seg_end = min(j_end, rv1);
    uint64_t p = run_pos[ri] + (j - rv0);
    uint64_t f = 0, r = 0;
    for (uint32_t i = 0; i < k; ++i) {
      f = srol1(f) ^ s_tab[32 + code[p + i]];
      r = srol1(r) ^ s_tab[32 + 3 - code[p + k - 1 - i]];
    }
    for (;;) {
      const uint64_t h = f + r;
      keys[key_phys(j)] = accepted(h) ? h : KEY_MAX;
      ++j;
      if (j >= seg_end) break;
      const uint32_t cout = code[p], cin = code[p + k];
      f = srol1(f) ^ s_tab[cin * 4 + cout];
      r = sror1(r ^ s_tab[16 + cin * 4 + cout]);
      ++p;
    }
    ++ri;
  }
}

__global__ __launch_bounds__(256) void k_keys_linear(const uint64_t* __restrict__ keys, uint64_t n, uint64_t* __restrict__ out)
{
  const uint64_t j = (uint64_t)blockIdx.x * blockDim.x + threadIdx.x;
  if (j < n) out[j] = keys[key_phys(j)];
}

struct WinParams
{
  const uint64_t* keys;
  const uint32_t* tile_ids;
  uint32_t n_tile_ids;
  const uint64_t* rec_vstart;
  const uint64_t* rec_nv;
  const uint64_t* tile_start;
  uint32_t n_rec;
  uint32_t w;
  uint32_t chunk;
  uint32_t levels;
  uint64_t* out_j;
  uint64_t* out_key;
  unsigned long long* seg_count;
  uint64_t seg_cap;
  uint32_t* tile_cnt;
  uint32_t tile_cap;
  const uint32_t* tile_any;
  const uint8_t* code;
  const uint64_t* run_pos;
  const uint64_t* run_vstart;
  uint32_t n_runs;
  HashParams hp;
  const uint32_t* bf;
  FastMod fm;
  uint64_t* dir_off;
  uint32_t* dir_cnt;
  uint32_t tile_base = 0;
};
constexpr uint32_t N_SEG = 64;
constexpr uint32_t WIN_FUSE_W = 64;
constexpr uint32_t WIN_FUSE_PER = (WIN_TILE + 1 + WIN_FUSE_W - 2 + WIN_THREADS - 1) / WIN_THREADS;

__device__ __forceinline__ uint32_t pe(uint32_t e)
{
  return e + (e >> 5);
}

__device__ __forceinline__ uint64_t win_key_slot(const WinParams& P, uint64_t tile)
{
  if (P.tile_ids == nullptr) return tile;
  uint32_t lo = 0, hi = P.n_tile_ids;
  while (hi - lo > 1) {
    const uint32_t mid = lo + ((hi - lo) >> 1);
    if (P.tile_ids[mid] <= tile)
      lo = mid;
    else
      hi = mid;
  }
  return lo;
}

__device__ __forceinline__ uint32_t better_idx(const uint64_t* s_key, uint32_t a, uint32_t b)
{
  const uint64_t ka = s_key[pe(a)], kb = s_key[pe(b)];
  if (ka < kb) return a;
  if (kb < ka) return b;
  return a > b ? a : b;
}

template <bool FUSED>
__global__ __launch_bounds__(WIN_THREADS) void k_window_min(WinParams P)
{
  extern __shared__ __attribute__((aligned(16))) unsigned char smem[];
  uint32_t lo = 0, hi = P.n_rec;
  const uint32_t blk = blockIdx.x + P.tile_base;
  const uint64_t b = blk;
  while (hi - lo > 1) {
    const uint32_t mid = lo + ((hi - lo) >> 1);
    if (P.tile_start[mid] <= b)
      lo = mid;
    else
      hi = mid;
  }
  const uint32_t rec = lo;
  const uint64_t nv = P.rec_nv[rec];
  const uint32_t w = P.w;
  const uint64_t n_win_rec = nv - w + 1;
  const uint64_t t0 = (b - P.tile_start[rec]) * (uint64_t)WIN_TILE;
  const uint32_t cnt = (uint32_t)min((uint64_t)WIN_TILE, n_win_rec - t0);
  const uint64_t tf = t0 > 0 ? t0 - 1 : 0;
  const uint32_t n_win = (uint32_t)(t0 + cnt - tf);
  const uint32_t E = n_win + w - 1;
  const uint32_t c = P.chunk;
  const uint32_t n_chunks = (E + c - 1) / c;

  const uint64_t ja = P.rec_vstart[rec] + tf, jb = ja + E;
  if (P.tile_any != nullptr) {
    bool any = false;
    for (uint64_t tile = ja / KEY_TILE; tile * KEY_TILE < jb; ++tile) any |= P.tile_any[tile] != 0;
    if (!any) return;
  }
  uint64_t* s_key = reinterpret_cast<uint64_t*>(smem);
  uint32_t* s_ctl = reinterpret_cast<uint32_t*>(s_key + pe(E) + 1);
  uint16_t* s_list = reinterpret_cast<uint16_t*>(s_ctl + 4);
  uint16_t* s_st = s_list + ((n_win + 8) & ~7u);
  if (threadIdx.x == 0) s_ctl[0] = 0;

  if (FUSED) {
    uint64_t* s_tab = reinterpret_cast<uint64_t*>((reinterpret_cast<uintptr_t>(s_st + (size_t)P.levels * n_chunks) + 15u) & ~(uintptr_t)15u);
    uint8_t* s_seq = reinterpret_cast<uint8_t*>(s_tab + 36);
    const uint32_t tid = threadIdx.x, k = P.hp.k;
    if (tid < 16) {
      s_tab[tid] = P.hp.roll_f[tid];
      s_tab[16 + tid] = P.hp.roll_r[tid];
    }
    if (tid < 4) s_tab[32 + tid] = P.hp.seed[tid];
    uint32_t rl = 0, rh = P.n_runs;
    while (rh - rl > 1) {
      const uint32_t mid = rl + ((rh - rl) >> 1);
      if (P.run_vstart[mid] <= ja)
        rl = mid;
      else
// ... 2617 lines not shown
  A.seg_cap = seg_cap;
  A.seg_count = d_ctl;
  A.tile_off = d_toff;
  A.tile_cnt = d_tcnt;
  A.tile_ordered = d_tord;
  ScopedTimer t(ctx, "bf_sparse_level", true);
  if (int rc_a = launch_accept(ctx, g, k, A, fold, n_kt)) return rc_a;
  HIP_TRY(ctx, hipGetLastError());
  unsigned long long counts[N_SEG];
  HIP_TRY(ctx, hipMemcpyAsync(counts, d_ctl, N_SEG * 8, hipMemcpyDeviceToHost, ctx->stream));
  HIP_TRY(ctx, hipStreamSynchronize(ctx->stream));
  uint64_t accepted = 0;
  for (uint32_t sgm = 0; sgm < N_SEG; ++sgm) {
    if (counts[sgm] > seg_cap) return 1;
    accepted += counts[sgm];
  }
  const uint64_t n16 = (acc->bytes + 15) / 16;
  const uint64_t n_gran = ((uint64_t)acc->bytes * 8 + (1ull << shift) - 1) >> shift;
  const uint64_t n_sw = (n_gran + 31) / 32;
  acc->popcnt = -1;
  ++acc->version;
  NTS_LAUNCH(k_bf_sparse_clear, dim3((uint32_t)std::min<uint64_t>((n_sw + 3) / 4, 256 * 16)), dim3(256), 0, ctx->stream, (uint4*)acc->d_words, n16,
                     acc->d_summary, n_sw, shift);
  HIP_TRY(ctx, hipMemsetAsync(acc->d_summary, 0, acc->summary_words * 4, ctx->stream));
  HIP_TRY(ctx, hipMemsetAsync(acc->d_fold, 0, 2 * FOLD_WORDS * 4, ctx->stream));
  NTS_LAUNCH(k_bf_sparse_set, dim3((uint32_t)((n_kt * 32 + 255) / 256)), dim3(256), 0, ctx->stream, acc->d_words, A.fm, d_sk, seg_cap, d_toff, d_tcnt,
                     n_kt, acc->d_summary, shift, acc->d_fold, d_ctl + N_SEG);
  HIP_TRY(ctx, hipGetLastError());
  unsigned long long n_set = 0;
  HIP_TRY(ctx, hipMemcpyAsync(&n_set, d_ctl + N_SEG, 8, hipMemcpyDeviceToHost, ctx->stream));
  HIP_TRY(ctx, hipStreamSynchronize(ctx->stream));
  acc->popcnt = (int64_t)n_set;
  acc->summary_shift = shift;
  acc->summary_version = acc->version;
  ctx->last_bf_sparse_level = 1;
  ctx->last_bf_sparse_accepted = accepted;
  return 0;
}

void launch_tiers(nts_ctx* ctx, const TierParams& Q, uint64_t n_tiles)
{
  const dim3 grid((uint32_t)n_tiles), block(TR_THREADS);
  if (Q.fm.form == 2)
    NTS_LAUNCH(k_hash_tiers<2>, grid, block, 0, ctx->stream, Q);
  else if (Q.fm.form == 1)
    NTS_LAUNCH(k_hash_tiers<1>, grid, block, 0, ctx->stream, Q);
  else
    NTS_LAUNCH(k_hash_tiers<0>, grid, block, 0, ctx->stream, Q);
}

__global__ void k_gap_tiers_ctl(const uint64_t* __restrict__ blk_scan_last, const uint64_t* __restrict__ blk_cnt_last, uint64_t n_sparse,
                                const unsigned long long* __restrict__ overflow, uint64_t* __restrict__ ctl)
{
  const uint64_t n = *blk_scan_last + *blk_cnt_last;
  const bool bad = *overflow != 0ULL;
  ctl[0] = bad ? 0 : n;
  ctl[1] = n_sparse + (bad ? 0 : n);
  ctl[2] = bad ? 1 : 0;
}

int tier_params(nts_ctx* ctx, const nts_genome* g, const GenomeTables& T, uint32_t k, uint32_t w, const nts_bf* filter, TierParams& Q)
{
  Q.pack = g->d_pack;
  Q.rec_vstart = T.d_rec_vstart;
  Q.n_rec = g->n_rec;
  Q.w = w;
  return genome_params(ctx, g, T, k, filter, Q);
}

SparseParams sparse_params(const uint64_t* pj, const uint64_t* pk, const uint64_t* tscan, const uint32_t* tcnt, uint64_t n_tiles, uint64_t m_max,
                           uint64_t n_valid, uint32_t w, uint64_t* stj, uint64_t* stk, uint64_t* bcnt, unsigned long long* ctl)
{
  SparseParams S;
  S.pj = pj;
  S.pk = pk;
  S.m_scan_last = tscan + (n_tiles - 1);
  S.m_cnt_last = tcnt + (n_tiles - 1);
  S.m_max = m_max;
  S.n_valid = n_valid;
  S.w = w;
  S.stage_j = stj;
  S.stage_k = stk;
  S.blk_cnt = bcnt;
  S.gap_count = ctl + N_SEG;
  S.overflow = ctl + N_SEG + 1;
  return S;
}

int run_gap_tiers(nts_ctx* ctx, const nts_genome* g, const GenomeTables& T, uint32_t k, uint32_t w, const nts_bf* filter, const SketchPlan& plan,
                  uint64_t tau, const std::vector<uint64_t>& pv, const std::vector<uint64_t>& pn, uint64_t covered, const SortedOut& sparse, SortedOut& res)
{
  res = SortedOut();
  if (!filter || k > FAST_K_MAX || w < 64 || w > 4097 || pv.empty() || ctx->gap_tiers_off) return NTS_OK;
  const uint32_t halo = ((w - 1 + 63) / 64) * 64, core = TR_EXT - 2 * halo;
  std::vector<TierTile> tiles;
  for (size_t i = 0; i < pv.size(); ++i) {
    const uint64_t a = pv[i], n = pn[i];
    if (n <= TR_EXT) {
      TierTile t = {};
      t.e0 = (int64_t)a;
      t.n = (uint32_t)n;
      t.c0 = 0;
      t.c1 = (uint32_t)n;
      t.flags = 3;
      tiles.push_back(t);
      continue;
    }
    for (uint64_t c_lo = 0; c_lo < n; c_lo += core) {
      const uint64_t e_lo = c_lo >= halo ? c_lo - halo : 0, e_hi = std::min<uint64_t>(n, c_lo + core + halo);
      TierTile t = {};
      t.e0 = (int64_t)(a + e_lo);
      t.n = (uint32_t)(e_hi - e_lo);
      t.c0 = (uint32_t)(c_lo - e_lo);
      t.c1 = (uint32_t)(std::min<uint64_t>(n, c_lo + core) - e_lo);
      t.flags = (e_lo == 0 ? 1u : 0u) | (e_hi == n ? 2u : 0u);
      tiles.push_back(t);
    }
  }
  const uint64_t n_gt = tiles.size();
  if (n_gt > (1u << 20)) return NTS_OK;
  void* dev[3];
  if (int rc = upload_packed(ctx, "gt_tables", { { tiles.data(), tiles.size() * sizeof(TierTile) }, { pv.data(), pv.size() * 8 }, { pn.data(), pn.size() * 8 } }, dev))
    return rc;
  const TierTile* d_tiles = (const TierTile*)dev[0];
  const uint64_t *d_vs = (const uint64_t*)dev[1], *d_nv = (const uint64_t*)dev[2];
  NTS_WS(d_dir, uint32_t*, "gt_dir", n_gt * 12);
  NTS_WS(d_toff, uint64_t*, "gt_tile_off", n_gt * 8);
  NTS_WS(d_tcnt, uint32_t*, "gt_tile_cnt", n_gt * 4 + 8);
  NTS_WS(d_tord, uint8_t*, "gt_tile_ord", n_gt);
  NTS_WS(d_tscan, uint64_t*, "gt_tile_scan", n_gt * 8);
  NTS_WS(d_ctl, unsigned long long*, "gt_ctl", (N_SEG + 4) * 8);
  const uint64_t tiles_per_seg = (n_gt + N_SEG - 1) / N_SEG;
  const uint64_t rich = std::min<uint64_t>(tiles_per_seg, 8) * (uint64_t)(core / 8 + 64);
  const uint64_t seg_cap = std::max<uint64_t>((uint64_t)((double)covered * 0.05 / N_SEG) + 2048, rich);
  const uint64_t m_max = seg_cap * N_SEG, n_blk = (m_max + SPARSE_BLOCK - 1) / SPARSE_BLOCK;
  NTS_WS(d_sj, uint64_t*, "gt_seg_j", m_max * 8);
  NTS_WS(d_sk, uint64_t*, "gt_seg_key", m_max * 8);
  NTS_WS(d_pj, uint64_t*, "gt_cand_j", m_max * 8);
  NTS_WS(d_pk, uint64_t*, "gt_cand_key", m_max * 8);
  NTS_WS(d_stj, uint64_t*, "gt_stage_j", n_blk * SPARSE_BLOCK * 8);
  NTS_WS(d_stk, uint64_t*, "gt_stage_k", n_blk * SPARSE_BLOCK * 8);
  NTS_WS(d_bcnt, uint64_t*, "gt_blk_cnt", n_blk * 8);
  NTS_WS(d_bscan, uint64_t*, "gt_blk_scan", n_blk * 8);
  NTS_WS(d_gj, uint64_t*, "gt_win_j", n_blk * SPARSE_BLOCK * 8);
  NTS_WS(d_gk, uint64_t*, "gt_win_key", n_blk * SPARSE_BLOCK * 8);
  NTS_WS(d_gctl, uint64_t*, "gap_ctl", 4 * 8);
  HIP_TRY(ctx, hipMemsetAsync(d_ctl, 0, (N_SEG + 4) * 8, ctx->stream));
  TierParams Q;
  if (int rc_q = tier_params(ctx, g, T, k, w, filter, Q)) return rc_q;
  Q.tiles = d_tiles;
  Q.excl_on = 1;
  Q.excl_hi = (uint32_t)(tau >> 32);
  Q.dir = d_dir;
  Q.halo = halo;
  Q.core = core;
  Q.scale = (float)(1.0 / ((double)(tau >> 32) + 1.0));
  Q.exp_shift = 23;
  Q.exp_bias = 127;
  uint32_t n_exp = 1;
  while (n_exp < TR_TIERS_MAX - 1 && (double)plan.c * (double)(2u << n_exp) <= 0.75 * (double)w) ++n_exp;
  Q.n_tiers = n_exp + 1;
  Q.seg_j = d_sj;
  Q.seg_key = d_sk;
  Q.seg_cap = seg_cap;
  Q.seg_count = d_ctl;
  Q.tile_off = d_toff;
  Q.tile_cnt = d_tcnt;
  Q.tile_ordered = d_tord;
  Q.stats = d_ctl + N_SEG + 2;
  Q.exp_stop = 0;
  {
    ScopedTimer t(ctx, "hash_probe");
    NTS_LAUNCH(k_tier_dir, dim3((uint32_t)((n_gt + 255) / 256)), dim3(256), 0, ctx->stream, T.d_run_vstart, T.n_runs, T.d_rec_vstart, g->n_rec,
                       T.rt.n_valid, halo, core, n_gt, d_tiles, d_dir);
    launch_tiers(ctx, Q, n_gt);
  }
  {
    ScopedTimer t(ctx, "window_min");
    if (int rc_s = scan_counts<uint32_t>(ctx, d_tcnt, n_gt, d_tscan)) return rc_s;
    NTS_LAUNCH(k_cand_compact, dim3((uint32_t)((n_gt + CC_TILES - 1) / CC_TILES)), dim3(256), 0, ctx->stream, d_sj, d_sk, seg_cap, d_toff, d_tcnt, d_tord,
                       d_tscan, n_gt, d_pj, d_pk, m_max, d_ctl + N_SEG + 1, false);
    SparseParams S = sparse_params(d_pj, d_pk, d_tscan, d_tcnt, n_gt, m_max, T.rt.n_valid, w, d_stj, d_stk, d_bcnt, d_ctl);
    S.rec_vstart = d_vs;
    S.rec_nv = d_nv;
    S.n_rec = (uint32_t)pv.size();
    S.gap_lo = S.gap_hi = nullptr;
    S.gap_cap = 0;
    S.rec_holes = 1;
    NTS_LAUNCH(k_sparse_win, dim3((uint32_t)n_blk), dim3(SPARSE_THREADS), 0, ctx->stream, S);
    if (int rc_s = scan_counts<uint64_t>(ctx, d_bcnt, n_blk, d_bscan)) return rc_s;
    NTS_LAUNCH(k_gather_winners, dim3((uint32_t)n_blk), dim3(256), 0, ctx->stream, d_stj, d_stk, d_bcnt, d_bscan, d_gj, d_gk);
    NTS_LAUNCH(k_gap_tiers_ctl, dim3(1), dim3(1), 0, ctx->stream, d_bscan + (n_blk - 1), d_bcnt + (n_blk - 1), sparse.count, d_ctl + N_SEG + 1, d_gctl);
  }
  HIP_TRY(ctx, hipGetLastError());
  res.d_j = sparse.d_j;
  res.d_key = sparse.d_key;
  res.na = sparse.count;
  res.b_j = d_gj;
  res.b_key = d_gk;
  res.count = sparse.count + std::min<uint64_t>(m_max, covered);
  res.d_ctl = d_gctl;
  return NTS_OK;
}

int run_pruned(nts_ctx* ctx, const nts_genome* g, const GenomeTables& T, uint32_t k, uint32_t w, const nts_bf* filter, const SketchPlan& plan,
               SortedOut& res)
{
  const RunTable& rt = T.rt;
  const uint64_t V = rt.n_valid;
  const uint32_t prune_c = plan.c;
  const bool tiers = plan.sel == SketchSel::Tiers, accept_list = plan.sel == SketchSel::AcceptList;
  const bool every_window = tiers || accept_list;
  const double hi_m4 = NTS_KNOB("NTS_HI_M4") ? atof(NTS_KNOB("NTS_HI_M4")) : 1.15, hi_m2 = NTS_KNOB("NTS_HI_M2") ? atof(NTS_KNOB("NTS_HI_M2")) : 1.2;
  const bool sel_hi = !every_window && ctx->select_impl != 1 && k <= HI_K_MAX && 4096.0 * prune_c / w * hi_m4 <= 256.0 &&
                      (ctx->select_impl == 2 || 2ull * T.n_runs <= (V + HIW_TILE - 1) / HIW_TILE + 64);
  const uint32_t hi_per = 4096.0 * prune_c / w * hi_m2 <= 128.0 ? 2u : 4u;
  const uint64_t sel_tile = tiers ? (uint64_t)plan.tiers.core : accept_list ? (uint64_t)KEY_TILE : sel_hi ? (uint64_t)HIW_TILE : (uint64_t)SEL_TILE;
  const uint64_t n_kt = (V + sel_tile - 1) / sel_tile;
  if (n_kt > 0x7FFFFFFFULL) return fail(ctx, NTS_ERANGE, "genome too large for one launch");
  const unsigned __int128 full = ((unsigned __int128)1) << 64;
  unsigned __int128 t128 = full / w * prune_c;
  uint64_t tau = t128 >= full - 1 ? KEY_MAX - 1 : ((uint64_t)t128 | 0xFFFFFFFFULL);
  if (tau == KEY_MAX) tau = KEY_MAX - 1;
  const double frac = accept_list ? 1.0 : std::min(1.0, (double)prune_c / (double)w);
  NTS_WS(d_toff, uint64_t*, "sel_tile_off", n_kt * 8);
  NTS_WS(d_tcnt, uint32_t*, "sel_tile_cnt", n_kt * 4 + 8);
  NTS_WS(d_tord, uint8_t*, "sel_tile_ord", n_kt);
  NTS_WS(d_tscan, uint64_t*, "sel_tile_scan", n_kt * 8);
  NTS_WS(d_ctl, unsigned long long*, "sel_ctl", (N_SEG + 2) * 8);
  const uint64_t gap_cap = V / w + g->n_rec + 16;
  NTS_WS(d_glo, uint64_t*, "gap_lo", gap_cap * 8);
  NTS_WS(d_ghi, uint64_t*, "gap_hi", gap_cap * 8);
  uint64_t cseg_cap = tiers ? (uint64_t)((double)V * (std::max(6.0, 2.5 * ctx->tier_x0) / (double)w + 0.002) * 1.25 / N_SEG) + 8192
                            : (uint64_t)((double)V * frac * std::min(1.0, 1.5 * plan.p + (accept_list ? 1e-4 : 0.02)) * 1.25 / N_SEG) + 8192;
  const bool elim_on = sel_hi && !(NTS_KNOB("NTS_SELECT_ELIM") && atoi(NTS_KNOB("NTS_SELECT_ELIM")) == 0);
  if (elim_on && !ctx->elim_needs_full_cap) cseg_cap = cseg_cap / 2 + 8192;
  unsigned long long ctl[N_SEG + 1];
  std::vector<uint64_t> glo(GAP_PEEK), ghi(GAP_PEEK);
  uint64_t m = 0, n_gap = 0, n_sparse = 0;
  uint64_t *d_sj = nullptr, *d_sk = nullptr;
  for (int attempt = 0; attempt < 2; ++attempt) {
    const uint64_t m_max = cseg_cap * N_SEG;
    const uint64_t n_blk = (m_max + SPARSE_BLOCK - 1) / SPARSE_BLOCK;
    const uint64_t slot_words = sel_hi ? n_kt * 64ull * hi_per : 0ull;
    d_sj = (uint64_t*)ws_get(ctx, "sel_seg_j", (slot_words + m_max) * 8);
    d_sk = (uint64_t*)ws_get(ctx, "sel_seg_key", (slot_words + m_max) * 8);
    NTS_WS(d_pj, uint64_t*, "cand_j", m_max * 8);
    NTS_WS(d_pk, uint64_t*, "cand_key", m_max * 8);
    NTS_WS(d_stj, uint64_t*, "stage_j", n_blk * SPARSE_BLOCK * 8);
    NTS_WS(d_stk, uint64_t*, "stage_k", n_blk * SPARSE_BLOCK * 8);
    NTS_WS(d_bcnt, uint64_t*, "blk_cnt", n_blk * 8);
    NTS_WS(d_bscan, uint64_t*, "blk_scan", n_blk * 8);
    if (!d_sj || !d_sk) return NTS_ENOMEM;
    if (!ctx->sel_ctl_clean) HIP_TRY(ctx, hipMemsetAsync(d_ctl, 0, (N_SEG + 2) * 8, ctx->stream));
    ctx->sel_ctl_clean = false;
    if (!accept_list) {
      if (int rc_pk = ensure_pack(ctx, g)) return rc_pk;
    }
    if (tiers) {
      const TierPlan& tp = plan.tiers;
      TierParams Q;
      if (int rc_q = tier_params(ctx, g, T, k, w, filter, Q)) return rc_q;
      NTS_WS(d_dir, uint32_t*, "tier_dir", n_kt * 12);
      NTS_WS(d_tstats, unsigned long long*, "tier_stats", 16);
      HIP_TRY(ctx, hipMemsetAsync(d_tstats, 0, 16, ctx->stream));
      Q.tiles = nullptr;
      Q.excl_on = Q.excl_hi = 0;
      Q.dir = d_dir;
      Q.halo = tp.halo;
      Q.core = tp.core;
      Q.scale = tp.scale;
      Q.exp_shift = tp.exp_shift;
      Q.exp_bias = tp.exp_bias;
      Q.n_tiers = tp.n_tiers;
      Q.seg_j = d_sj;
      Q.seg_key = d_sk;
      Q.seg_cap = cseg_cap;
      Q.seg_count = d_ctl;
      Q.tile_off = d_toff;
      Q.tile_cnt = d_tcnt;
      Q.tile_ordered = d_tord;
      Q.stats = d_tstats;
      Q.exp_stop = NTS_KNOB("NTS_TR_STOP") ? (uint32_t)atoi(NTS_KNOB("NTS_TR_STOP")) : 0u;
      ScopedTimer t(ctx, "hash_tiers", true);
      NTS_LAUNCH(k_tier_dir, dim3((uint32_t)((n_kt + 255) / 256)), dim3(256), 0, ctx->stream, T.d_run_vstart, T.n_runs, T.d_rec_vstart, g->n_rec, V,
                         tp.halo, tp.core, n_kt, (const TierTile*)nullptr, d_dir);
      launch_tiers(ctx, Q, n_kt);
    } else if (accept_list) {
      AcceptParams A;
      if (int rc_gp = genome_params(ctx, g, T, k, filter, A)) return rc_gp;
      A.summary = plan.summary;
      A.shift = plan.summary_shift;
      A.probe_mask = ~0u;
#ifdef NTS_EXPERIMENTS
      if (NTS_KNOB("NTS_ACC_NO_LOOKUP") && atoi(NTS_KNOB("NTS_ACC_NO_LOOKUP"))) {
        A.probe_mask = 0u;
        static std::once_flag warned;
        std::call_once(warned, [] { fprintf(stderr, "[ntsynt_hip] NTS_ACC_NO_LOOKUP is set: sparse-filter sketches return WRONG results (timing experiment only)\n"); });
      }
#endif
      A.seg_j = d_sj;
      A.seg_key = d_sk;
      A.seg_cap = cseg_cap;
      A.seg_count = d_ctl;
      A.tile_off = d_toff;
      A.tile_cnt = d_tcnt;
      A.tile_ordered = d_tord;
      ScopedTimer t(ctx, "hash_accept", true);
      if (int rc_a = launch_accept(ctx, g, k, A, plan.fold, n_kt)) return rc_a;
    } else {
      SelParams S;
      if (int rc_gp = genome_params(ctx, g, T, k, filter, S)) return rc_gp;
      S.pack = g->d_pack;
      S.tau = tau;
      S.seg_j = d_sj;
      S.seg_key = d_sk;
      S.seg_cap = cseg_cap;
      S.seg_count = d_ctl;
      S.tile_off = d_toff;
      S.tile_cnt = d_tcnt;
      S.tile_ordered = d_tord;
      S.w_elim = (NTS_KNOB("NTS_SELECT_ELIM") && atoi(NTS_KNOB("NTS_SELECT_ELIM")) == 0) ? 0u : w;
      const bool chained = g_live_contexts.load() > 1 && ctx->device < 32 && !(NTS_KNOB("NTS_SELECT_CHAIN") && atoi(NTS_KNOB("NTS_SELECT_CHAIN")) == 0);
      std::unique_lock<std::mutex> chain_lock(nts_chain::mu, std::defer_lock);
      if (chained) {
        chain_lock.lock();
        if (nts_chain::live[ctx->device]) HIP_TRY(ctx, hipStreamWaitEvent(ctx->stream, nts_chain::ev[ctx->device], 0));
      }
      struct ChainRecord
      {
        nts_ctx* c;
        bool on;
        ~ChainRecord()
        {
          if (!on) return;
          hipEvent_t& e = nts_chain::ev[c->device];
          if (!e && hipEventCreateWithFlags(&e, hipEventDisableTiming) != hipSuccess) return;
          if (hipEventRecord(e, c->stream) == hipSuccess) nts_chain::live[c->device] = true;
        }
      } chain_record{ ctx, chained };
      ScopedTimer t(ctx, filter ? "hash_select" : "hash_select_nofilter", true);
      {
        const uint32_t slots = 64.0 * frac > 2.5 ? 16u : 8u;
        const uint32_t need = (uint32_t)std::min(16.0, std::ceil(48.0 * frac + 4.0));
        S.flush_at = slots == 8 ? 8u : slots - need;
      }
      const uint32_t nch = (k + 3) / 4;
      if (sel_hi) {
        const uint64_t waves_wanted = 256ull * 32ull * 2ull;
        uint32_t tpw = (uint32_t)std::min<uint64_t>(16, std::max<uint64_t>(1, n_kt / waves_wanted));
        if (const char* e = NTS_KNOB("NTS_HI_TPW")) tpw = (uint32_t)std::max(1, std::min(64, atoi(e)));
        const uint64_t per_wg = (uint64_t)HIW_WAVES * tpw;
        const dim3 grid((uint32_t)((n_kt + per_wg - 1) / per_wg));
        if (filter && hi_per == 2)
          NTS_LAUNCH((k_hash_select_hi<true, 2>), grid, dim3(HIW_THREADS), nch * 4096u, ctx->stream, S, nch, tpw, n_kt);
        else if (filter)
          NTS_LAUNCH((k_hash_select_hi<true, 4>), grid, dim3(HIW_THREADS), nch * 4096u, ctx->stream, S, nch, tpw, n_kt);
        else if (hi_per == 2)
          NTS_LAUNCH((k_hash_select_hi<false, 2>), grid, dim3(HIW_THREADS), nch * 4096u, ctx->stream, S, nch, tpw, n_kt);
        else
          NTS_LAUNCH((k_hash_select_hi<false, 4>), grid, dim3(HIW_THREADS), nch * 4096u, ctx->stream, S, nch, tpw, n_kt);
      }
      else if (64.0 * frac > 2.5)
        NTS_LAUNCH(k_hash_select<16>, dim3((uint32_t)n_kt), dim3(HASH_THREADS), 0, ctx->stream, S);
      else
        NTS_LAUNCH(k_hash_select<8>, dim3((uint32_t)n_kt), dim3(HASH_THREADS), 0, ctx->stream, S);
    }
    {
      ScopedTimer t(ctx, "cand_compact");
      if (int rc_s = scan_counts<uint32_t>(ctx, d_tcnt, n_kt, d_tscan)) return rc_s;
      if (sel_hi)
        NTS_LAUNCH(k_cand_compact_slots, dim3((uint32_t)((n_kt + CCS_TILES - 1) / CCS_TILES)), dim3(256), 0, ctx->stream, d_sj, d_sk, d_toff, d_tcnt, d_tscan, n_kt,
                           d_pj, d_pk, m_max, d_ctl + N_SEG + 1);
      else
        NTS_LAUNCH(k_cand_compact, dim3((uint32_t)((n_kt + CC_TILES - 1) / CC_TILES)), dim3(256), 0, ctx->stream, d_sj, d_sk, cseg_cap, d_toff, d_tcnt, d_tord, d_tscan, n_kt,
                           d_pj, d_pk, m_max, d_ctl + N_SEG + 1, false);
    }
    SparseParams Q = sparse_params(d_pj, d_pk, d_tscan, d_tcnt, n_kt, m_max, V, w, d_stj, d_stk, d_bcnt, d_ctl);
    Q.rec_vstart = T.d_rec_vstart;
    Q.rec_nv = T.d_rec_nv;
    Q.n_rec = g->n_rec;
    Q.gap_lo = d_glo;
    Q.gap_hi = d_ghi;
    Q.gap_cap = gap_cap;
    Q.no_gaps = every_window ? 1u : 0u;
    {
      ScopedTimer t(ctx, "sparse_win");
      NTS_LAUNCH(k_sparse_win, dim3((uint32_t)n_blk), dim3(SPARSE_THREADS), 0, ctx->stream, Q);
      if (int rc_s = scan_counts<uint64_t>(ctx, d_bcnt, n_blk, d_bscan)) return rc_s;
    }
    HIP_TRY(ctx, hipGetLastError());
    uint64_t last_scan = 0, last_cnt = 0, listed = 0;
    {
      static_assert(N_SEG + 7 + 2 * GAP_PEEK < MAIL_WORDS - 8, "mailbox too small (the last word is the arrival flag)");
      const uint32_t peek = (uint32_t)std::min<uint64_t>(GAP_PEEK, gap_cap);
      Mail mb(ctx);
      const uint32_t a_ctl = mb.add(d_ctl, N_SEG + 1);
      const uint32_t a_scan = mb.add(d_bscan + (n_blk - 1), 1);
      const uint32_t a_cnt = mb.add(d_bcnt + (n_blk - 1), 1);
      const uint32_t a_tscan = mb.add(d_tscan + (n_kt - 1), 1);
      const uint32_t a_tcnt = mb.add((const uint64_t*)(d_tcnt + ((n_kt - 1) & ~1ull)), 1);
      const uint32_t a_lo = mb.add(d_glo, peek, d_ctl + N_SEG);
      const uint32_t a_hi = mb.add(d_ghi, peek, d_ctl + N_SEG);
      const uint32_t a_tier = tiers ? mb.add((const uint64_t*)ws_get(ctx, "tier_stats", 16), 2) : 0u;
      int rc_m = mb.launch(ctx);
      if (rc_m) return rc_m;
      {
        ScopedTimer t(ctx, "gather_winners");
        NTS_LAUNCH(k_gather_winners, dim3((uint32_t)n_blk), dim3(256), 0, ctx->stream, d_stj, d_stk, d_bcnt, d_bscan, d_sj, d_sk);
      }
      HIP_TRY(ctx, hipGetLastError());
      if ((rc_m = mb.wait(ctx))) return rc_m;
      for (uint32_t i = 0; i <= N_SEG; ++i) ctl[i] = ctx->mail[a_ctl + i];
      last_scan = ctx->mail[a_scan];
      last_cnt = ctx->mail[a_cnt];
      listed = ctx->mail[a_tscan] + (uint32_t)(ctx->mail[a_tcnt] >> (32 * ((n_kt - 1) & 1ull)));
      memcpy(glo.data(), ctx->mail + a_lo, (size_t)peek * 8);
      memcpy(ghi.data(), ctx->mail + a_hi, (size_t)peek * 8);
      if (tiers) {
        ctx->last_tier_probes = ctx->mail[a_tier];
        ctx->last_tier_rounds = ctx->mail[a_tier + 1];
      }
    }
    uint64_t worst = 0;
    m = 0;
    for (uint32_t s = 0; s < N_SEG; ++s) {
      worst = std::max<uint64_t>(worst, ctl[s]);
      m += ctl[s];
    }
    n_gap = ctl[N_SEG];
    n_sparse = last_scan + last_cnt;
    ctx->last_many_listed = sel_hi ? m : 0;
    if (sel_hi) {
      m = listed;
      if (listed > m_max) worst = std::max<uint64_t>(worst, listed / N_SEG + 1);
    }
    if (NTS_KNOB("NTS_DEBUG_RETRY")) fprintf(stderr, "[select] attempt %d: worst segment %llu of %llu, listed %llu, tiers %d\n", attempt, (unsigned long long)worst, (unsigned long long)cseg_cap, (unsigned long long)m, tiers ? 1 : 0);
    if (worst <= cseg_cap) break;
    if (elim_on) ctx->elim_needs_full_cap = true;
    if (attempt == 1) return fail(ctx, NTS_EHIP, "candidate segments overflowed twice");
    cseg_cap = worst + 1024;
  }
  ctx->last_candidates = m;
  if (every_window) n_gap = 0;
  ctx->last_gaps = n_gap;
  res.d_j = d_sj;
  res.d_key = d_sk;
  res.count = n_sparse;
  if (n_gap == 0) return NTS_OK;
  if (n_gap > gap_cap) return fail(ctx, NTS_EHIP, "uncovered-range list overflowed");
  if (n_gap > GAP_PEEK) {
    glo.resize(n_gap);
    ghi.resize(n_gap);
    HIP_TRY(ctx, hipMemcpyAsync(glo.data(), d_glo, n_gap * 8, hipMemcpyDeviceToHost, ctx->stream));
    HIP_TRY(ctx, hipMemcpyAsync(ghi.data(), d_ghi, n_gap * 8, hipMemcpyDeviceToHost, ctx->stream));
    HIP_TRY(ctx, hipStreamSynchronize(ctx->stream));
  }
  std::vector<size_t> ord(n_gap);
  for (size_t i = 0; i < n_gap; ++i) ord[i] = i;
  std::sort(ord.begin(), ord.end(), [&](size_t a, size_t b) { return glo[a] < glo[b]; });
  std::vector<uint64_t> pv(n_gap), pn(n_gap);
  std::vector<uint32_t> tiles, spans;
  uint64_t covered = 0;
  for (size_t i = 0; i < n_gap; ++i) {
    const uint64_t a = glo[ord[i]], b = ghi[ord[i]];
    pv[i] = a;
    pn[i] = b - a + 1;
    covered += pn[i];
    for (uint64_t t = a / KEY_TILE; t <= b / KEY_TILE; ++t) {
      const uint32_t lo_in = (uint32_t)(std::max(a, t * KEY_TILE) - t * KEY_TILE);
      const uint32_t hi_in = (uint32_t)(std::min(b, t * KEY_TILE + KEY_TILE - 1) - t * KEY_TILE);
      if (tiles.empty() || tiles.back() != (uint32_t)t) {
        tiles.push_back((uint32_t)t);
        spans.push_back(lo_in);
        spans.push_back(hi_in);
      } else {
        spans[spans.size() - 1] = std::max(spans.back(), hi_in);
      }
    }
  }
  ctx->last_gap_kmers = covered;
  SortedOut dense;
  SortedOut sparse_list;
  sparse_list.d_j = d_sj;
  sparse_list.d_key = d_sk;
  sparse_list.count = n_sparse;
  if (plan.few_ranges) {
    int rc_g = run_gap_tiers(ctx, g, T, k, w, filter, plan, tau, pv, pn, covered, sparse_list, dense);
    if (rc_g) return rc_g;
    if (dense.d_ctl) {
      res = dense;
      return NTS_OK;
    }
  }
  int rc = run_dense_sorted(ctx, g, T, k, w, filter, plan, &pv, &pn, &tiles, covered, "gap_", dense, &sparse_list, &spans);
  if (rc) return rc;
  if (dense.d_ctl) {
    res = dense;
    return NTS_OK;
  }
  if (dense.count == 0) return NTS_OK;
  const uint64_t total = n_sparse + dense.count;
  NTS_WS(d_mj, uint64_t*, "merged_j", total * 8);
  NTS_WS(d_mk, uint64_t*, "merged_key", total * 8);
  {
    ScopedTimer t(ctx, "merge_lists");
    NTS_LAUNCH(k_merge_lists, dim3((uint32_t)((total + 255) / 256)), dim3(256), 0, ctx->stream, d_sj, d_sk, n_sparse, dense.d_j, dense.d_key,
                       dense.count, d_mj, d_mk);
  }
  HIP_TRY(ctx, hipGetLastError());
  res.d_j = d_mj;
  res.d_key = d_mk;
  res.count = total;
  return NTS_OK;
}

int plan_sketch(nts_ctx* ctx, const nts_genome* g, const GenomeTables& T, uint32_t k, uint32_t w, const nts_bf* filter, const nts_bf* filter_out,
                SketchPlan& plan)
// ... 78 lines not shown
    uint32_t shift = 7;
    const uint32_t sum_log2 = NTS_KNOB("NTS_SUMMARY_LOG2_BITS") ? (uint32_t)std::max(16, std::min(28, atoi(NTS_KNOB("NTS_SUMMARY_LOG2_BITS")))) : SUMMARY_LOG2_BITS;
    while ((bits / (double)(1ull << shift)) > (double)(1ull << sum_log2) && shift < 30) ++shift;
    const double sum_max = NTS_KNOB("NTS_SUMMARY_MAX") ? atof(NTS_KNOB("NTS_SUMMARY_MAX")) : (plan.sel == SketchSel::Tiers ? 0.7 : 3.0);
    if ((double)pc / bits * (double)(1ull << shift) < sum_max) {
      if (int rc = bf_make_summary(ctx, filter, shift)) return rc;
      const uint64_t key_tiles = (rt.n_valid + KEY_TILE - 1) / KEY_TILE;
      NTS_WS(d_any, uint32_t*, "tile_any", (key_tiles + 4) * 4);
      plan.summary = filter->d_summary;
      plan.summary_shift = shift;
      plan.tile_any = d_any;
      const double own = bits * (1.0 - std::exp(-(double)rt.n_valid / bits));
      plan.p = own > 0 ? std::min(1.0, (double)pc / own) : 1.0;
      if (ctx->sketch_mode != 1) plan.sel = SketchSel::AcceptList;
      plan.fold = (ctx->fold_mode == 0 && bits >= (double)(1u << FOLD_BITS_LOG2) && (double)pc < 1.2 * (double)(1u << FOLD_BITS_LOG2))
                    ? filter->d_fold : nullptr;
    }
  }
  return NTS_OK;
}

}

extern "C" int nts_sketch_mode(nts_ctx* ctx, int mode, uint32_t prune_c)
{
  if (!ctx || mode < 0 || mode > 2) return fail(ctx, NTS_EINVAL, "nts_sketch_mode: mode must be 0 (auto), 1 (dense) or 2 (pruned)");
  ctx->sketch_mode = mode;
  ctx->prune_c = prune_c;
  return NTS_OK;
}

extern "C" int nts_sketch_summary(nts_ctx* ctx, int mode, uint32_t* last_shift)
{
  if (!ctx || mode < -1 || mode > 2) return fail(ctx, NTS_EINVAL, "nts_sketch_summary: mode is -1 (query), 0 (auto), 1 (never) or 2 (no LDS copy)");
  if (mode >= 0) {
    ctx->summary_mode = mode == 1 ? 1 : 0;
    ctx->fold_mode = mode == 2 ? 1 : 0;
  }
  if (last_shift) *last_shift = ctx->last_summary;
  return NTS_OK;
}

extern "C" int nts_sketch_select(nts_ctx* ctx, int impl)
{
  if (!ctx || impl < 0 || impl > 2)
    return fail(ctx, NTS_EINVAL, "nts_sketch_select: impl is 0 (auto), 1 (full-width rolling) or 2 (upper halves wherever the kernel applies)");
  ctx->select_impl = impl;
  return NTS_OK;
}

extern "C" int nts_sketch_tiers(nts_ctx* ctx, int mode, double x0, int half_steps, uint64_t* last_probes, uint64_t* last_rounds, uint32_t* last_tiers)
{
  if (!ctx || mode < -1 || mode > 2 || x0 < 0 || x0 > 64)
    return fail(ctx, NTS_EINVAL, "nts_sketch_tiers: mode is -1 (query), 0 (auto), 1 (never) or 2 (wherever the kernel applies); 0 <= x0 <= 64");
  if (mode >= 0) {
    ctx->tier_mode = mode;
    ctx->gap_tiers_off = mode == 1 ? 1 : 0;
    ctx->tier_x0 = x0;
    ctx->tier_half = half_steps ? 1u : 0u;
  }
  if (last_probes) *last_probes = ctx->last_tier_probes;
  if (last_rounds) *last_rounds = ctx->last_tier_rounds;
  if (last_tiers) *last_tiers = (uint32_t)ctx->last_tiers;
  return NTS_OK;
}

extern "C" int nts_path_stats(nts_ctx* ctx, uint64_t* sketch_many_listed, uint64_t* bf_direct_indices, uint32_t* bf_list_fallback)
{
  if (!ctx) return NTS_EINVAL;
  if (sketch_many_listed) *sketch_many_listed = ctx->last_many_listed;
  if (bf_direct_indices) *bf_direct_indices = ctx->last_bf_direct;
  if (bf_list_fallback) *bf_list_fallback = ctx->last_bf_fallback;
  return NTS_OK;
}

extern "C" int nts_bf_level_stats(nts_ctx* ctx, uint32_t* sparse_level, uint64_t* accepted_kmers)
{
  if (!ctx) return NTS_EINVAL;
  if (sparse_level) *sparse_level = ctx->last_bf_sparse_level;
  if (accepted_kmers) *accepted_kmers = ctx->last_bf_sparse_accepted;
  return NTS_OK;
}

extern "C" int nts_sketch_stats(nts_ctx* ctx, uint64_t* candidates, uint64_t* uncovered_ranges, uint64_t* uncovered_kmers, uint32_t* prune_c_used)
{
  if (!ctx) return NTS_EINVAL;
  if (prune_c_used) *prune_c_used = ctx->last_c;
  if (candidates) *candidates = ctx->last_candidates;
  if (uncovered_ranges) *uncovered_ranges = ctx->last_gaps;
  if (uncovered_kmers) *uncovered_kmers = ctx->last_gap_kmers;
  return NTS_OK;
}

extern "C" int nts_sketch(nts_ctx* ctx, const nts_genome* g, uint32_t k, uint32_t w, const nts_bf* filter, const nts_interval* mask,
                          uint64_t n_mask, nts_mx** out)
{
  return nts_sketch_ex(ctx, g, k, w, filter, nullptr, mask, n_mask, out);
}

extern "C" int nts_sketch_ex(nts_ctx* ctx, const nts_genome* g, uint32_t k, uint32_t w, const nts_bf* filter, const nts_bf* filter_out,
                             const nts_interval* mask, uint64_t n_mask, nts_mx** out)
{
  if (!ctx || !g || !out || k == 0 || w == 0 || (n_mask && !mask)) return fail(ctx, NTS_EINVAL, "nts_sketch: bad arguments");
  if (w > WIN_MAX_W) return fail(ctx, NTS_ERANGE, "nts_sketch: w exceeds the LDS-resident window limit (12000)");
  HIP_TRY(ctx, hipSetDevice(ctx->device));
  GenomeTables scratch;
  const GenomeTables* T = nullptr;
  int rc = get_tables(ctx, g, k, mask, n_mask, scratch, &T);
  if (rc) return rc;
  const RunTable& rt = T->rt;
  nts_mx* mx = new nts_mx();
  ctx->last_candidates = ctx->last_gaps = ctx->last_gap_kmers = ctx->last_many_listed = 0;
  if (rt.n_valid == 0 || T->n_win_tiles(w) == 0) {
    *out = mx;
    return NTS_OK;
  }
  auto bail = [&](int code) {
    hipStreamSynchronize(ctx->stream);
    nts_mx_free(ctx, mx);
    return code;
  };
#define SK_TRY(expr)                                                                                \
  do {                                                                                              \
    int rc_ = (expr);                                                                               \
    if (rc_ != NTS_OK) return bail(rc_);                                                            \
  } while (0)
#define SK_HIP(expr)                                                                                \
  do {                                                                                              \
    hipError_t e_ = (expr);                                                                         \
    if (e_ != hipSuccess) {                                                                         \
      ctx->err = std::string(#expr) + ": " + hipGetErrorString(e_);                                 \
      return bail(e_ == hipErrorOutOfMemory ? NTS_ENOMEM : NTS_EHIP);                               \
    }                                                                                               \
  } while (0)
#define SK_WS(ptr, type, name, bytes)                                                               \
  type ptr = (type)ws_get(ctx, name, bytes);                                                        \
  if (!ptr) return bail(NTS_ENOMEM)

  SketchPlan plan;
  SK_TRY(plan_sketch(ctx, g, *T, k, w, filter, filter_out, plan));
  ctx->last_c = plan.c;
  ctx->last_tiers = plan.sel == SketchSel::Tiers ? plan.tiers.n_tiers : 0;
  ctx->last_tier_probes = ctx->last_tier_rounds = 0;
  ctx->last_summary = plan.summary ? plan.summary_shift : 0;

  for (int attempt = 0;; ++attempt) {
    SortedOut res;
    if (plan.sel != SketchSel::Dense) {
      const int rc_p = run_pruned(ctx, g, *T, k, w, filter, plan, res);
      if (rc_p == NTS_ENOMEM && plan.sel == SketchSel::Tiers && w < WIN_FUSE_W) {
        plan.sel = SketchSel::Dense;
        plan.c = 0;
        ctx->last_c = ctx->last_tiers = 0;
        SK_TRY(run_dense_sorted(ctx, g, *T, k, w, filter, plan, nullptr, nullptr, nullptr, rt.n_valid, "", res));
      } else {
        SK_TRY(rc_p);
      }
    } else
      SK_TRY(run_dense_sorted(ctx, g, *T, k, w, filter, plan, nullptr, nullptr, nullptr, rt.n_valid, "", res));
    const uint64_t count = res.count;
    mx->n = count;
    if (count) {
      SK_TRY(alloc_result(ctx, mx, count));
      {
        const uint64_t n_first = res.b_j ? res.na : count;
        const uint64_t n_chunks = n_first / FIN_CHUNK + 1;
        SK_WS(d_cb, uint64_t*, "fin_chunks", n_chunks * 16);
        uint32_t* const d_crun = (uint32_t*)(d_cb + n_chunks);
        uint32_t* const d_crec = d_crun + n_chunks;
        ScopedTimer t(ctx, "finalize");
        NTS_LAUNCH(k_fin_chunks, dim3((uint32_t)((n_chunks + 255) / 256)), dim3(256), 0, ctx->stream, res.d_j, n_first,
                           res.d_ctl ? res.d_ctl + 1 : nullptr, res.b_j, res.b_j ? res.d_ctl : nullptr, T->d_run_pos, T->d_run_vstart, T->n_runs,
                           g->d_rec_off, g->n_rec, d_cb, d_crun, d_crec);
        NTS_LAUNCH(k_finalize, dim3((uint32_t)((count + 255) / 256)), dim3(256), 0, ctx->stream, res.d_j, res.d_key, (uint64_t)count,
                           res.d_ctl ? res.d_ctl + 1 : nullptr, res.b_j, res.b_key, res.b_j ? res.d_ctl : nullptr, res.na, T->d_run_pos, T->d_run_vstart, T->n_runs, g->d_rec_off, g->n_rec, k,
                           d_cb, d_crun, d_crec, mx->d_h1, mx->d_rec, mx->d_pos);
      }
      SK_HIP(hipGetLastError());
    }
    uint64_t* const sel_ctl = plan.sel != SketchSel::Dense ? (uint64_t*)ws_get(ctx, "sel_ctl", (N_SEG + 2) * 8) : nullptr;
    if (!res.d_ctl) {
      Mail done(ctx);
      if (sel_ctl) done.clear_after(sel_ctl, N_SEG + 2);
      SK_TRY(done.post(ctx));
      ctx->sel_ctl_clean = sel_ctl != nullptr;
      break;
    }
    Mail mb(ctx);
    const uint32_t at = mb.add(res.d_ctl, 3);
    if (sel_ctl) mb.clear_after(sel_ctl, N_SEG + 2);
    SK_TRY(mb.post(ctx));
    ctx->sel_ctl_clean = sel_ctl != nullptr;
    if (ctx->mail[at + 2] == 0) {
      mx->n = ctx->mail[at + 1];
      break;
    }
    if (attempt == 1) return bail(fail(ctx, NTS_EHIP, "nts_sketch: uncovered ranges could not be merged"));
    ctx->mx_pool.push_back({ mx->d_h1, mx->cap_bytes });
    mx->d_h1 = nullptr;
    mx->d_pos = nullptr;
    mx->d_rec = nullptr;
    plan.few_ranges = false;
  }
  *out = mx;
  return NTS_OK;
#undef SK_TRY
#undef SK_HIP
#undef SK_WS
}

extern "C" {

uint64_t nts_mx_count(const nts_mx* mx)
{
  return mx ? mx->n : 0;
}

void nts_mx_free(nts_ctx* ctx, nts_mx* mx)
{
  if (!mx) return;
  if (ctx) hipSetDevice(ctx->device);
  if (mx->d_h1) {
    if (ctx && ctx->mx_pool.size() < 32 && mx->cap_bytes)
      ctx->mx_pool.push_back({ mx->d_h1, mx->cap_bytes });
    else
      dev_free(mx->d_h1);
  }
  delete mx;
}

int nts_mx_download(nts_ctx* ctx, const nts_mx* mx, uint64_t* h1, uint32_t* rec, uint64_t* pos)
{
  if (!ctx || !mx) return fail(ctx, NTS_EINVAL, "nts_mx_download: bad arguments");
  if (mx->n == 0) return NTS_OK;
  if (!h1 || !rec || !pos) return fail(ctx, NTS_EINVAL, "nts_mx_download: NULL output");
  HIP_TRY(ctx, hipSetDevice(ctx->device));
  HIP_TRY(ctx, hipMemcpyAsync(h1, mx->d_h1, mx->n * 8, hipMemcpyDeviceToHost, ctx->stream));
  HIP_TRY(ctx, hipMemcpyAsync(rec, mx->d_rec, mx->n * 4, hipMemcpyDeviceToHost, ctx->stream));
  HIP_TRY(ctx, hipMemcpyAsync(pos, mx->d_pos, mx->n * 8, hipMemcpyDeviceToHost, ctx->stream));
  HIP_TRY(ctx, hipStreamSynchronize(ctx->stream));
  return NTS_OK;
}

int nts_mx_export_async(nts_ctx* ctx, const nts_mx* mx, void* h1_dev, void* rec_dev, void* pos_dev)
{
  if (!ctx || !mx) return fail(ctx, NTS_EINVAL, "nts_mx_export: bad arguments");
  if (mx->n == 0) return NTS_OK;
  if (!h1_dev || !rec_dev || !pos_dev) return fail(ctx, NTS_EINVAL, "nts_mx_export: NULL destination");
  HIP_TRY(ctx, hipSetDevice(ctx->device));
  HIP_TRY(ctx, hipMemcpyAsync(h1_dev, mx->d_h1, mx->n * 8, hipMemcpyDeviceToDevice, ctx->stream));
  HIP_TRY(ctx, hipMemcpyAsync(rec_dev, mx->d_rec, mx->n * 4, hipMemcpyDeviceToDevice, ctx->stream));
  HIP_TRY(ctx, hipMemcpyAsync(pos_dev, mx->d_pos, mx->n * 8, hipMemcpyDeviceToDevice, ctx->stream));
  return NTS_OK;
}

int nts_mx_export(nts_ctx* ctx, const nts_mx* mx, void* h1_dev, void* rec_dev, void* pos_dev)
{
  const int rc = nts_mx_export_async(ctx, mx, h1_dev, rec_dev, pos_dev);
  if (rc != NTS_OK || mx->n == 0) return rc;
  HIP_TRY(ctx, hipStreamSynchronize(ctx->stream));
  return NTS_OK;
}

int nts_mx_device_ptrs(const nts_mx* mx, void** h1, void** rec, void** pos)
{
  if (!mx) return NTS_EINVAL;
  if (h1) *h1 = mx->d_h1;
  if (rec) *rec = mx->d_rec;
  if (pos) *pos = mx->d_pos;
  return NTS_OK;
}

int nts_mx_upload(nts_ctx* ctx, const uint64_t* h1, const uint32_t* rec, const uint64_t* pos, uint64_t n, nts_mx** out)
// ... 32 lines not shown
```

ntsynt_amd/device.py:

```python
import ctypes
import os

import numpy as np

from . import _lib
from ._lib import Interval, c_vp, u64


class NtsError(RuntimeError):
    pass


MEM_EVENT_NAMES = ("driver_calls", "ns_in_driver_calls", "served_from_cache", "retried_after_emptying_the_cache", "bytes_from_driver",
                   "bytes_to_driver", "ns_waiting_for_device_before_keeping_a_block", "reserve_calls")


def mem_events(lib):
    out = (ctypes.c_uint64 * 8)()
    lib.nts_mem_events(out)
    return dict(zip(MEM_EVENT_NAMES, [int(x) for x in out]))


def mem_events_since(lib, before):
    now = mem_events(lib)
# ... 50 lines not shown
            raise ValueError("minhash_pairs: sketches [n, s], one count per row, pair lists of one length")
        shared = np.zeros(a.size, dtype=np.uint32)
        size = np.zeros(a.size, dtype=np.uint32)
        self.check(self.lib.nts_minhash_pairs(self.h, sk.shape[1], sk.ctypes.data, cnt.ctypes.data, sk.shape[0], a.ctypes.data, b.ctypes.data,
                                              a.size, shared.ctypes.data, size.ctypes.data), "nts_minhash_pairs")
        return shared, size

    def iv_links(self, lists, min_anchors):
        arrs = [np.ascontiguousarray(a, dtype=SAMPLE_DTYPE) for a in lists]
        assert SAMPLE_DTYPE.itemsize == ctypes.sizeof(_lib.Sample) and LINK_DTYPE.itemsize == ctypes.sizeof(_lib.IvLink)
        ptrs = (c_vp * max(len(arrs), 1))(*[a.ctypes.data for a in arrs])
        counts = np.array([a.size for a in arrs], dtype=np.uint64)
        p, n = c_vp(), u64()
        self.check(self.lib.nts_iv_links(self.h, len(arrs), ptrs, counts.ctypes.data_as(_lib.c_u64p), int(min_anchors), ctypes.byref(p),
                                         ctypes.byref(n)), "nts_iv_links")
        out = np.empty(n.value, dtype=LINK_DTYPE)
        if n.value:
            ctypes.memmove(out.ctypes.data, p.value, out.nbytes)
        self.lib.nts_free(p)
        return out

    def iv_sites(self, lists, target, step, min_hits):
        arrs = [np.ascontiguousarray(a, dtype=SAMPLE_DTYPE) for a in lists]
        tgt = np.ascontiguousarray(target, dtype=SAMPLE_DTYPE)
        assert SAMPLE_DTYPE.itemsize == ctypes.sizeof(_lib.Sample) and SITE_DTYPE.itemsize == ctypes.sizeof(_lib.IvSite)
        ptrs = (c_vp * max(len(arrs), 1))(*[a.ctypes.data for a in arrs])
        counts = np.array([a.size for a in arrs], dtype=np.uint64)
        p, n = c_vp(), u64()
        self.check(self.lib.nts_iv_sites(self.h, len(arrs), ptrs, counts.ctypes.data_as(_lib.c_u64p), tgt.ctypes.data if tgt.size else None, tgt.size,
                                         int(step), int(min_hits), ctypes.byref(p), ctypes.byref(n)), "nts_iv_sites")
        out = np.empty(n.value, dtype=SITE_DTYPE)
        if n.value:
            ctypes.memmove(out.ctypes.data, p.value, out.nbytes)
        self.lib.nts_free(p)
        return out

    def iv_periods(self, records, n_iv):
        rec = np.ascontiguousarray(records, dtype=SAMPLE_DTYPE)
        assert SAMPLE_DTYPE.itemsize == ctypes.sizeof(_lib.Sample) and PERIOD_DTYPE.itemsize == ctypes.sizeof(_lib.IvPeriod)
        out = np.zeros(int(n_iv), dtype=PERIOD_DTYPE)
        self.check(self.lib.nts_iv_periods(self.h, rec.ctypes.data if rec.size else None, rec.size, int(n_iv), out.ctypes.data if out.size else None),
                   "nts_iv_periods")
        return out

    def timing(self, name):
        ms, n = ctypes.c_double(), u64()
        self.check(self.lib.nts_timing(self.h, name.encode(), ctypes.byref(ms), ctypes.byref(n)), "nts_timing")
        return ms.value, n.value

    def sketch_mode(self, mode="auto", prune_c=0):
        code = {"auto": 0, "dense": 1, "pruned": 2}[mode]
        self.check(self.lib.nts_sketch_mode(self.h, code, int(prune_c)), "nts_sketch_mode")
        self._sketch_mode = (mode, int(prune_c))

    def sketch_summary(self, mode=None):
        last = ctypes.c_uint32()
        code = {None: -1, "auto": 0, "never": 1, "no-lds": 2}[mode]
        self.check(self.lib.nts_sketch_summary(self.h, code, ctypes.byref(last)), "nts_sketch_summary")
        return last.value

    def sketch_select(self, impl="auto"):
        self.check(self.lib.nts_sketch_select(self.h, {"auto": 0, "full": 1, "hi": 2}[impl]), "nts_sketch_select")

    def sketch_tiers(self, mode=None, x0=0.0, half_steps=False):
        a, b, c = u64(), u64(), ctypes.c_uint32()
        code = {None: -1, "auto": 0, "never": 1, "always": 2}[mode]
        self.check(self.lib.nts_sketch_tiers(self.h, code, float(x0), int(bool(half_steps)), ctypes.byref(a), ctypes.byref(b), ctypes.byref(c)),
                   "nts_sketch_tiers")
        return a.value, b.value, c.value

    def bf_build_mode(self, mode="auto"):
        self.check(self.lib.nts_bf_build_mode(self.h, {"auto": 0, "atomic": 1, "binned": 2}[mode]), "nts_bf_build_mode")

    def sketch_stats(self):
        a, b, c, d = u64(), u64(), u64(), ctypes.c_uint32()
        self.check(self.lib.nts_sketch_stats(self.h, ctypes.byref(a), ctypes.byref(b), ctypes.byref(c), ctypes.byref(d)),
                   "nts_sketch_stats")
        self.last_prune_c = d.value
        return a.value, b.value, c.value

    def path_stats(self):
        a, b, c = u64(), u64(), ctypes.c_uint32()
        self.check(self.lib.nts_path_stats(self.h, ctypes.byref(a), ctypes.byref(b), ctypes.byref(c)), "nts_path_stats")
        return {"sketch_many_listed": a.value, "bf_direct_indices": b.value, "bf_list_fallback": c.value}

    def bf_level_stats(self):
        a, b = ctypes.c_uint32(), u64()
        self.check(self.lib.nts_bf_level_stats(self.h, ctypes.byref(a), ctypes.byref(b)), "nts_bf_level_stats")
        return {"sparse_level": a.value, "accepted_kmers": b.value}

    VALU_KINDS = ["v_xor_b32", "v_alignbit_b32", "v_lshl_add_u64", "v_lshlrev_b64", "v_mul_lo_u32", "v_mad_u64_u32",
                  "v_add_co_u32+v_addc_co_u32", "v_xor_b32 (dependent chain)", "v_add3_u32", "v_cmp_ge_u32+v_addc_co_u32",
                  "roll31 step (9 instructions)"]

    def bench_valu(self, kind, waves_per_simd=4, iters=20000):
        ms, cyc, n = ctypes.c_double(), ctypes.c_double(), ctypes.c_double()
        k = self.VALU_KINDS.index(kind) if isinstance(kind, str) else int(kind)
        self.check(self.lib.nts_bench_valu(self.h, k, int(waves_per_simd), int(iters), ctypes.byref(ms), ctypes.byref(cyc),
                                           ctypes.byref(n)), "nts_bench_valu")
        per_cu = 4 * waves_per_simd * n.value / (ms.value * 1e-3)
        return {"instruction": self.VALU_KINDS[k], "waves_per_simd": int(waves_per_simd), "wall_ms": round(ms.value, 4),
                "cycles_per_wave_instr_per_simd": round(cyc.value, 3), "wave_instr_per_s_per_cu": per_cu,
                "implied_clock_GHz": round(per_cu * cyc.value / 4 / 1e9, 3)}

    def set_graph_budget(self, nbytes):
        self.check(self.lib.nts_graph_budget(self.h, int(nbytes)), "nts_graph_budget")

    def graph_last_plan(self):
        v, e, o, p = ctypes.c_uint32(), ctypes.c_uint32(), ctypes.c_uint32(), u64()
        self.check(self.lib.nts_graph_last_plan(self.h, ctypes.byref(v), ctypes.byref(e), ctypes.byref(p), ctypes.byref(o)),
                   "nts_graph_last_plan")
        return {"v_slices": v.value, "e_slices": e.value, "scratch_peak": p.value, "oversize": o.value}

    def mem_stats(self):
        a, b, c, d = u64(), u64(), u64(), u64()
        self.check(self.lib.nts_mem_stats(self.h, ctypes.byref(a), ctypes.byref(b), ctypes.byref(c), ctypes.byref(d)), "nts_mem_stats")
        return {"live": a.value, "peak": b.value, "device_used": c.value, "device_total": d.value}

    def alloc_stats(self):
        n, ms = u64(), ctypes.c_double()
        self.lib.nts_alloc_stats(ctypes.byref(n), ctypes.byref(ms))
        return n.value, ms.value

    def mem_trim(self):
        return int(self.lib.nts_mem_trim())

    def mem_cache_stats(self):
        a, b = u64(), u64()
        self.lib.nts_mem_cache_stats(ctypes.byref(a), ctypes.byref(b))
        return a.value, b.value

    def mem_reset_peak(self):
        self.lib.nts_mem_reset_peak()

    def mem_reserve(self, nbytes):
        got = u64()
        self.check(self.lib.nts_mem_reserve(self.device, int(nbytes), ctypes.byref(got)), "nts_mem_reserve")
        return got.value

    def mem_reserve_async(self, nbytes):
        import threading
        box = {"got": 0}

        def work():
            try:
                box["got"] = self.mem_reserve(nbytes)
            except Exception:
                box["got"] = 0
        th = threading.Thread(target=work, name="nts_mem_reserve", daemon=True)
        th.start()

        class _Pending:
            def join(self_inner):
                th.join()
                return box["got"]
        return _Pending()

    def mem_events(self):
        return mem_events(self.lib)

    def mem_events_since(self, before):
        return mem_events_since(self.lib, before)

    def trim_ingest(self):
        self.check(self.lib.nts_ingest_trim(self.h), "nts_ingest_trim")

    def trim_bf_build(self):
# ... 623 lines not shown
```

Baseline: 1529.

## Decide sparse windows directly from per-wave select slots, skipping candidate compaction

Adds a direct path in which the select kernel records per-wave candidate counts, and a new slot-based window kernel reads candidates straight from each wave's slot region with neighbouring halos. This skips the scan and compaction pass into cand_j/cand_key. When a window needs data beyond the halo, or a wave spilled candidates to segments, it sets a general flag, and the host retries on the old path and disables direct mode for later calls. The aim is to save a kernel launch, a scan and a global read/write pass, at the cost of a possible redo.

After: 1463. 0.957x the previous value.

```diff
diff --git a/include/ntsynt_hip.h b/include/ntsynt_hip.h
--- a/include/ntsynt_hip.h
+++ b/include/ntsynt_hip.h
@@ -150,6 +150,7 @@
 int nts_sketch_tiers(nts_ctx* ctx, int mode, double x0, int half_steps, uint64_t* last_probes, uint64_t* last_rounds, uint32_t* last_tiers);
 int nts_sketch_stats(nts_ctx* ctx, uint64_t* candidates, uint64_t* uncovered_ranges, uint64_t* uncovered_kmers, uint32_t* prune_c_used);
 int nts_path_stats(nts_ctx* ctx, uint64_t* sketch_many_listed, uint64_t* bf_direct_indices, uint32_t* bf_list_fallback);
+int nts_win_direct_stats(nts_ctx* ctx, uint32_t* used_by_last_sketch, uint32_t* given_up);
 int nts_bf_level_stats(nts_ctx* ctx, uint32_t* sparse_level, uint64_t* accepted_kmers);
 uint64_t nts_mx_count(const nts_mx* mx);
 void nts_mx_free(nts_ctx* ctx, nts_mx* mx);
diff --git a/ntsynt_amd/_lib.py b/ntsynt_amd/_lib.py
--- a/ntsynt_amd/_lib.py
+++ b/ntsynt_amd/_lib.py
@@ -151,6 +151,7 @@
     ("nts_sketch_tiers", ctypes.c_int, [c_vp, ctypes.c_int, ctypes.c_double, ctypes.c_int, ctypes.c_void_p, ctypes.c_void_p, ctypes.c_void_p]),
     ("nts_sketch_stats", ctypes.c_int, [c_vp, c_u64p, c_u64p, c_u64p, c_u32p]),
     ("nts_path_stats", ctypes.c_int, [c_vp, c_u64p, c_u64p, c_u32p]),
+    ("nts_win_direct_stats", ctypes.c_int, [c_vp, c_u32p, c_u32p]),
     ("nts_bf_level_stats", ctypes.c_int, [c_vp, c_u32p, c_u64p]),
     ("nts_mx_count", u64, [c_vp]),
     ("nts_mx_free", None, [c_vp, c_vp]),
diff --git a/ntsynt_amd/csrc/nts_internal.h b/ntsynt_amd/csrc/nts_internal.h
--- a/ntsynt_amd/csrc/nts_internal.h
+++ b/ntsynt_amd/csrc/nts_internal.h
@@ -445,6 +445,8 @@
   std::vector<IoLane> io_up, io_down;
   double dense_seg_per_window = 3.0;
   double fused_seg_per_window = 2.5;
+  bool win_direct_off = false;
+  bool last_win_direct = false;
   bool elim_needs_full_cap = false;
   int select_impl = 0;
   int summary_mode = 0;
diff --git a/ntsynt_amd/csrc/nts_pruned.inc b/ntsynt_amd/csrc/nts_pruned.inc
--- a/ntsynt_amd/csrc/nts_pruned.inc
+++ b/ntsynt_amd/csrc/nts_pruned.inc
@@ -27,6 +27,7 @@
   uint32_t* tile_cnt;
   uint8_t* tile_ordered;
   uint32_t w_elim;
+  uint32_t* wave_cnt = nullptr;
 };
 
 
@@ -664,6 +665,7 @@
     }
   };
   uint32_t wave_run = 0;
+  uint32_t wave_elsewhere = 0;
   auto finish_pending = [&]() {
     if (pd_tile == ~0ULL) return;
     uint32_t okm = pd_m;
@@ -908,6 +910,7 @@
           if (lane == 0) base = listed_ok ? atomicAdd(&P.seg_count[seg], (unsigned long long)listed_ok) : 0ULL;
           base = __shfl(base, 0, 64);
           fits = base + listed_ok <= P.seg_cap;
+          if (listed_ok) wave_elsewhere = 1;
           if (listed_ok == 0 || !fits) break;
         }
         uint64_t dst = n_tiles * HIW_LIST + (uint64_t)seg * P.seg_cap + base;
@@ -955,6 +958,7 @@
   issue_probes();
   wait_probes();
   finish_pending();
+  if (lane == 0) P.wave_cnt[(uint64_t)blk * HIW_WAVES + wv] = wave_run | (wave_elsewhere << 24);
 }
 
 __global__ __launch_bounds__(256) void k_cand_compact(const uint64_t* __restrict__ seg_j, const uint64_t* __restrict__ seg_key,
@@ -1132,6 +1136,145 @@
 constexpr uint32_t SPARSE_HALO = 64;
 constexpr uint32_t SPARSE_REC_LDS = 2048;
 
+template <bool DIRECT>
+__device__ __forceinline__ uint32_t sparse_decide(const SparseParams& P, const ulonglong2* s_c, const uint64_t* s_rv, uint32_t* s_wcnt, bool recs_in_lds,
+                                                  uint32_t n_st, uint32_t own_lo, uint32_t own_n, bool more_left, bool more_right, uint64_t i0, uint64_t m,
+                                                  uint64_t lds_lo, uint64_t stage_at, uint32_t stage_room, unsigned long long* general)
+{
+  const uint64_t lds_hi = lds_lo + n_st;
+  auto cand_j = [&](uint64_t q) -> uint64_t { return (q >= lds_lo && q < lds_hi) ? s_c[q - lds_lo].x : P.pj[q]; };
+  auto cand_k = [&](uint64_t q) -> uint64_t { return (q >= lds_lo && q < lds_hi) ? s_c[q - lds_lo].y : P.pk[q]; };
+  const uint32_t lane = threadIdx.x & 63u, wv = threadIdx.x >> 6;
+  uint32_t winners_so_far = 0;
+  for (uint32_t item = 0; item < SPARSE_ITEMS; ++item) {
+  const uint32_t own_i = item * SPARSE_THREADS + threadIdx.x;
+  const uint64_t i = i0 + own_i;
+  bool win = false;
+  uint64_t j = 0, key = 0;
+  if (own_i < own_n) {
+    const uint32_t li = own_lo + own_i;
+    j = s_c[li].x;
+    key = s_c[li].y;
+    uint32_t lo = 0, hi = P.n_rec;
+    if (recs_in_lds) {
+      while (hi - lo > 1) {
+        const uint32_t mid = lo + ((hi - lo) >> 1);
+        if (s_rv[mid] <= j)
+          lo = mid;
+        else
+          hi = mid;
+      }
+    } else {
+      while (hi - lo > 1) {
+        const uint32_t mid = lo + ((hi - lo) >> 1);
+        if (P.rec_vstart[mid] <= j)
+          lo = mid;
+        else
+          hi = mid;
+      }
+    }
+    uint64_t rs, re;
+    if (recs_in_lds) {
+      rs = s_rv[lo];
+      re = lo + 1 < P.n_rec ? s_rv[lo + 1] : P.n_valid;
+    } else {
+      rs = P.rec_vstart[lo];
+      re = rs + P.rec_nv[lo];
+    }
+    const uint64_t w = P.w;
+    if (re - rs >= w) {
+      const uint64_t a_lim = (j - rs >= w - 1) ? j - (w - 1) : rs;
+      const uint64_t b_lim = (re - 1 - j >= w - 1) ? j + (w - 1) : re - 1;
+      uint64_t a_min = a_lim, b_max = b_lim;
+      bool redo_left = more_left, redo_right = more_right;
+      {
+        constexpr uint32_t STOPPED = 0x80000000u;
+        uint32_t ql = li, qr = li;
+        for (;;) {
+          const bool gl = ql - 1u < STOPPED - 1u;
+          const bool gr = qr + 1u < n_st;
+          if (!(gl | gr)) break;
+          const uint32_t il = ql - (gl ? 1u : 0u), ir = qr + (gr ? 1u : 0u);
+          const ulonglong2 L = s_c[min(il, n_st - 1u)], R = s_c[min(ir, n_st - 1u)];
+          ql = (gl & ((L.x < a_lim) | (L.y < key))) ? (il | STOPPED) : il;
+          qr = (gr & ((R.x > b_lim) | (R.y <= key))) ? (ir | STOPPED) : ir;
+        }
+        if (ql & STOPPED) {
+          const uint64_t x = s_c[ql & ~STOPPED].x;
+          if (x >= a_lim) a_min = x + 1;
+        }
+        if (qr & STOPPED) {
+          const uint64_t x = s_c[qr & ~STOPPED].x;
+          if (x <= b_lim) b_max = x - 1;
+        }
+        redo_left = redo_left & (ql == 0u);
+        redo_right = redo_right & (qr + 1u == n_st);
+      }
+      if (DIRECT) {
+        if (redo_left | redo_right) *general = 1ULL;
+      } else {
+        if (redo_left) {
+          a_min = a_lim;
+          for (uint64_t q = i; q-- > 0;) {
+            const uint64_t jq = cand_j(q);
+            if (jq < a_lim) break;
+            if (cand_k(q) < key) {
+              a_min = jq + 1;
+              break;
+            }
+          }
+        }
+        if (redo_right) {
+          b_max = b_lim;
+          for (uint64_t q = i + 1; q < m; ++q) {
+            const uint64_t jq = cand_j(q);
+            if (jq > b_lim) break;
+            if (cand_k(q) <= key) {
+              b_max = jq - 1;
+              break;
+            }
+          }
+        }
+      }
+      bool have_next = false;
+      uint64_t j_next = 0;
+      if (li + 1 < n_st) {
+        j_next = s_c[li + 1].x;
+        have_next = j_next < re;
+      }
+      win = b_max - a_min + 1 >= w;
+      const uint64_t nxt = have_next ? j_next : re;
+      if (!P.no_gaps) {
+        if (nxt - j - 1 >= w) push_gap(P, j + 1, nxt - 1);
+        const bool first_in_rec = (li == 0) || (s_c[li - 1].x < rs);
+        if (first_in_rec && j - rs >= w) push_gap(P, rs, j - 1);
+      }
+    }
+  }
+  const unsigned long long bal = __ballot(win);
+  if (item) __syncthreads();
+  if (lane == 0) s_wcnt[wv] = (uint32_t)__popcll(bal);
+  __syncthreads();
+  uint32_t base = 0, total = 0;
+  for (uint32_t q = 0; q < SPARSE_THREADS / 64; ++q) {
+    const uint32_t c = s_wcnt[q];
+    if (q < wv) base += c;
+    total += c;
+  }
+  if (win) {
+    const uint32_t r = winners_so_far + base + (uint32_t)__popcll(bal & ((1ULL << lane) - 1ULL));
+    if (DIRECT && r >= stage_room) {
+      *general = 1ULL;
+    } else {
+      P.stage_j[stage_at + r] = j;
+      P.stage_k[stage_at + r] = key;
+    }
+  }
+  winners_so_far += total;
+  }
+  return winners_so_far;
+}
+
 __global__ __launch_bounds__(SPARSE_THREADS) void k_sparse_win(SparseParams P)
 {
   __shared__ uint32_t s_wcnt[SPARSE_THREADS / 64];
@@ -1166,128 +1309,135 @@
   if (recs_in_lds)
     for (uint32_t q = threadIdx.x; q < P.n_rec; q += SPARSE_THREADS) s_rv[q] = P.rec_vstart[q];
   __syncthreads();
-  auto cand_j = [&](uint64_t q) -> uint64_t { return (q >= lds_lo && q < lds_hi) ? s_c[q - lds_lo].x : P.pj[q]; };
-  auto cand_k = [&](uint64_t q) -> uint64_t { return (q >= lds_lo && q < lds_hi) ? s_c[q - lds_lo].y : P.pk[q]; };
-  const uint32_t lane = threadIdx.x & 63u, wv = threadIdx.x >> 6;
-  uint32_t winners_so_far = 0;
-  for (uint32_t item = 0; item < SPARSE_ITEMS; ++item) {
-  const uint64_t i = blk0 + (uint64_t)item * SPARSE_THREADS + threadIdx.x;
-  bool win = false;
-  uint64_t j = 0, key = 0;
-  if (i < m) {
-    j = cand_j(i);
-    key = cand_k(i);
-    uint32_t lo = 0, hi = P.n_rec;
-    if (recs_in_lds) {
-      while (hi - lo > 1) {
-        const uint32_t mid = lo + ((hi - lo) >> 1);
-        if (s_rv[mid] <= j)
-          lo = mid;
-        else
-          hi = mid;
-      }
-    } else {
-      while (hi - lo > 1) {
-        const uint32_t mid = lo + ((hi - lo) >> 1);
-        if (P.rec_vstart[mid] <= j)
-          lo = mid;
-        else
-          hi = mid;
-      }
-    }
-    uint64_t rs, re;
-    if (recs_in_lds) {
-      rs = s_rv[lo];
-      re = lo + 1 < P.n_rec ? s_rv[lo + 1] : P.n_valid;
-    } else {
-      rs = P.rec_vstart[lo];
-      re = rs + P.rec_nv[lo];
-    }
-    const uint64_t w = P.w;
-    if (re - rs >= w) {
-      const uint64_t a_lim = (j - rs >= w - 1) ? j - (w - 1) : rs;
-      const uint64_t b_lim = (re - 1 - j >= w - 1) ? j + (w - 1) : re - 1;
-      uint64_t a_min = a_lim, b_max = b_lim;
-      const uint32_t li = (uint32_t)(i - lds_lo), n_st = (uint32_t)(lds_hi - lds_lo);
-      bool redo_left = lds_lo > 0, redo_right = lds_hi < m;
-      {
-        constexpr uint32_t STOPPED = 0x80000000u;
-        uint32_t ql = li, qr = li;
-        for (;;) {
-          const bool gl = ql - 1u < STOPPED - 1u;
-          const bool gr = qr + 1u < n_st;
-          if (!(gl | gr)) break;
-          const uint32_t il = ql - (gl ? 1u : 0u), ir = qr + (gr ? 1u : 0u);
-          const ulonglong2 L = s_c[min(il, n_st - 1u)], R = s_c[min(ir, n_st - 1u)];
-          ql = (gl & ((L.x < a_lim) | (L.y < key))) ? (il | STOPPED) : il;
-          qr = (gr & ((R.x > b_lim) | (R.y <= key))) ? (ir | STOPPED) : ir;
-        }
-        if (ql & STOPPED) {
-          const uint64_t x = s_c[ql & ~STOPPED].x;
-          if (x >= a_lim) a_min = x + 1;
-        }
-        if (qr & STOPPED) {
-          const uint64_t x = s_c[qr & ~STOPPED].x;
-          if (x <= b_lim) b_max = x - 1;
-        }
-        redo_left = redo_left & (ql == 0u);
-        redo_right = redo_right & (qr + 1u == n_st);
-      }
-      if (redo_left) {
-        a_min = a_lim;
-        for (uint64_t q = i; q-- > 0;) {
-          const uint64_t jq = cand_j(q);
-          if (jq < a_lim) break;
-          if (cand_k(q) < key) {
-            a_min = jq + 1;
-            break;
-          }
-        }
-      }
-      if (redo_right) {
-        b_max = b_lim;
-        for (uint64_t q = i + 1; q < m; ++q) {
-          const uint64_t jq = cand_j(q);
-          if (jq > b_lim) break;
-          if (cand_k(q) <= key) {
-            b_max = jq - 1;
-            break;
-          }
-        }
-      }
-      bool have_next = false;
-      uint64_t j_next = 0;
-      if (i + 1 < m) {
-        j_next = s_c[li + 1].x;
-        have_next = j_next < re;
-      }
-      win = b_max - a_min + 1 >= w;
-      const uint64_t nxt = have_next ? j_next : re;
-      if (!P.no_gaps) {
-        if (nxt - j - 1 >= w) push_gap(P, j + 1, nxt - 1);
-        const bool first_in_rec = (i == 0) || (s_c[li - 1].x < rs);
-        if (first_in_rec && j - rs >= w) push_gap(P, rs, j - 1);
-      }
-    }
-  }
-  const unsigned long long bal = __ballot(win);
-  if (item) __syncthreads();
-  if (lane == 0) s_wcnt[wv] = (uint32_t)__popcll(bal);
+  const uint32_t winners = sparse_decide<false>(P, s_c, s_rv, s_wcnt, recs_in_lds, (uint32_t)(lds_hi - lds_lo), (uint32_t)(blk0 - lds_lo),
+                                                (uint32_t)min((uint64_t)SPARSE_BLOCK, m - blk0), lds_lo > 0, lds_hi < m, blk0, m, lds_lo, blk0, SPARSE_BLOCK,
+                                                nullptr);
+  if (threadIdx.x == 0) P.blk_cnt[blockIdx.x] = winners;
+}
+
+constexpr uint32_t SLOT_WALK = 64;
+constexpr uint32_t SLOT_G_MAX = 64;
+constexpr uint32_t SLOT_REC_LDS = SPARSE_REC_LDS - 128;
+
+struct SlotParams
+{
+  const uint64_t* seg_j;
+  const uint64_t* seg_key;
+  const uint32_t* wave_cnt;
+  const uint64_t* tile_off;
+  const uint32_t* tile_cnt;
+  uint64_t n_tiles;
+  uint32_t n_waves;
+  uint32_t region;
+  uint32_t G, S;
+  unsigned long long* ctl;
+};
+
+__global__ __launch_bounds__(SPARSE_THREADS) void k_sparse_win_slots(SparseParams P, SlotParams D)
+{
+  __shared__ uint32_t s_wcnt[SPARSE_THREADS / 64];
+  __shared__ ulonglong2 s_c[SPARSE_BLOCK + 2 * SPARSE_HALO];
+  __shared__ uint64_t s_rv[SLOT_REC_LDS];
+  __shared__ uint32_t s_ex[3][64];
+  __shared__ uint32_t s_tot[3];
+  const uint32_t tid = threadIdx.x, lane = tid & 63u, wv = tid >> 6;
+  unsigned long long* const general = D.ctl + SEL_CTL_GENERAL;
+  const int64_t first = (int64_t)blockIdx.x * D.G;
+  if (!P.no_gaps)
+    for (uint64_t r = (uint64_t)blockIdx.x * SPARSE_THREADS + tid; r < P.n_rec; r += (uint64_t)gridDim.x * SPARSE_THREADS) {
+      const uint64_t rs = P.rec_vstart[r], nv = P.rec_nv[r];
+      if (nv < P.w) continue;
+      const uint64_t t0 = rs / HIW_TILE, t1 = (rs + nv - 1) / HIW_TILE;
+      bool found = false;
+      for (uint64_t t = t0; t <= t1 && t < D.n_tiles && !found; ++t) {
+        const uint32_t n = D.tile_cnt[t];
+        if (!n) continue;
+        const uint64_t off = D.tile_off[t];
+        if (off == ~0ULL || (t != t0 && t != t1)) {
+          found = true;
+          break;
+        }
+        uint32_t lo = 0, hi = n;
+        while (lo < hi) {
+          const uint32_t mid = lo + ((hi - lo) >> 1);
+          if (D.seg_j[off + mid] < rs)
+            lo = mid + 1;
+          else
+            hi = mid;
+        }
+        found = lo < n && D.seg_j[off + lo] < rs + nv;
+      }
+      if (!found) push_gap(P, rs, rs + nv - 1);
+    }
+  uint32_t cnt = 0, elsewhere = 0;
+  if (wv < 3) {
+    const int64_t wi = wv == 0 ? first - (int64_t)SLOT_WALK + lane : wv == 1 ? first + lane : first + D.G + lane;
+    if (wi >= 0 && wi < (int64_t)D.n_waves && (wv != 1 || lane < D.G)) {
+      const uint32_t word = D.wave_cnt[wi];
+      cnt = min(word & 0xFFFFFFu, D.region);
+      elsewhere = wv == 1 ? word >> 24 : 0u;
+    }
+  }
+  const bool recs_in_lds = P.n_rec <= SLOT_REC_LDS && !P.rec_holes;
+  if (recs_in_lds)
+    for (uint32_t q = tid; q < P.n_rec; q += SPARSE_THREADS) s_rv[q] = P.rec_vstart[q];
+  uint32_t incl = cnt;
+#pragma unroll
+  for (uint32_t d = 1; d < 64; d <<= 1) {
+    const uint32_t up = (uint32_t)__shfl_up((int)incl, d, 64);
+    if (lane >= d) incl += up;
+  }
+  if (wv < 3) {
+    s_ex[wv][lane] = incl - cnt;
+    if (lane == 63) s_tot[wv] = incl;
+  }
+  if (__any(elsewhere != 0u) && lane == 0) *general = 1ULL;
   __syncthreads();
-  uint32_t base = 0, total = 0;
-  for (uint32_t q = 0; q < SPARSE_THREADS / 64; ++q) {
-    const uint32_t c = s_wcnt[q];
-    if (q < wv) base += c;
-    total += c;
-  }
-  if (win) {
-    const uint32_t r = winners_so_far + base + (uint32_t)__popcll(bal & ((1ULL << lane) - 1ULL));
-    P.stage_j[blk0 + r] = j;
-    P.stage_k[blk0 + r] = key;
-  }
-  winners_so_far += total;
-  }
-  if (threadIdx.x == 0) P.blk_cnt[blockIdx.x] = winners_so_far;
+  const uint32_t T0 = s_tot[0], n = s_tot[1], T2 = s_tot[2];
+  const uint32_t blk_first = blockIdx.x * D.S;
+  if (n == 0) {
+    if (tid < D.S) P.blk_cnt[blk_first + tid] = 0;
+    return;
+  }
+  if (tid == 0) {
+    atomicAdd(D.ctl + SEL_CTL_LISTED, (unsigned long long)n);
+    if ((T0 == 0 && first > (int64_t)SLOT_WALK) || (T2 == 0 && first + D.G + SLOT_WALK < (int64_t)D.n_waves)) *general = 1ULL;
+  }
+  auto entry_at = [&](uint32_t q) -> uint64_t {
+    const uint32_t g = q < T0 ? 0u : q < T0 + n ? 1u : 2u;
+    const uint32_t qq = q - (g == 0 ? 0u : g == 1 ? T0 : T0 + n);
+    const uint32_t* const ex = s_ex[g];
+    uint32_t lo = 0, hi = 64;
+    while (hi - lo > 1) {
+      const uint32_t mid = lo + ((hi - lo) >> 1);
+      if (ex[mid] <= qq)
+        lo = mid;
+      else
+        hi = mid;
+    }
+    const int64_t wi = (g == 0 ? first - (int64_t)SLOT_WALK : g == 1 ? first : first + D.G) + lo;
+    return (uint64_t)wi * D.region + (qq - ex[lo]);
+  };
+  const uint32_t all = T0 + n + T2;
+  const uint32_t room = D.S * SPARSE_BLOCK;
+  uint32_t winners = 0;
+  for (uint32_t c0 = 0; c0 < n; c0 += SPARSE_BLOCK) {
+    const uint32_t own_at = T0 + c0, own_n = min(SPARSE_BLOCK, n - c0);
+    const uint32_t lo = own_at >= SPARSE_HALO ? own_at - SPARSE_HALO : 0u;
+    const uint32_t hi = min(all, own_at + own_n + SPARSE_HALO);
+    if (c0) __syncthreads();
+    for (uint32_t q = lo + tid; q < hi; q += SPARSE_THREADS) {
+      const uint64_t at = entry_at(q);
+      s_c[q - lo] = make_ulonglong2(D.seg_j[at], D.seg_key[at]);
+    }
+    __syncthreads();
+    winners += sparse_decide<true>(P, s_c, s_rv, s_wcnt, recs_in_lds, hi - lo, own_at - lo, own_n, lo > 0, hi < all, 0, 0, 0,
+                                   (uint64_t)blk_first * SPARSE_BLOCK + winners, winners < room ? room - winners : 0u, general);
+  }
+  if (tid < D.S) {
+    const uint32_t at = tid * SPARSE_BLOCK;
+    P.blk_cnt[blk_first + tid] = winners > at ? min(SPARSE_BLOCK, winners - at) : 0u;
+  }
 }
 
 __global__ __launch_bounds__(256) void k_gather_winners(const uint64_t* __restrict__ stage_j, const uint64_t* __restrict__ stage_k,
diff --git a/ntsynt_amd/csrc/ntsynt_hip.hip b/ntsynt_amd/csrc/ntsynt_hip.hip
--- a/ntsynt_amd/csrc/ntsynt_hip.hip
+++ b/ntsynt_amd/csrc/ntsynt_hip.hip
@@ -500,6 +500,11 @@
   uint32_t tile_base = 0;
 };
 constexpr uint32_t N_SEG = 64;
+constexpr uint32_t SEL_CTL_GAPS = N_SEG;
+constexpr uint32_t SEL_CTL_OVERFLOW = N_SEG + 1;
+constexpr uint32_t SEL_CTL_LISTED = N_SEG + 2;
+constexpr uint32_t SEL_CTL_GENERAL = N_SEG + 3;
+constexpr uint32_t SEL_CTL_WORDS = N_SEG + 4;
 constexpr uint32_t WIN_FUSE_W = 64;
 constexpr uint32_t WIN_FUSE_PER = (WIN_TILE + 1 + WIN_FUSE_W - 2 + WIN_THREADS - 1) / WIN_THREADS;
 
@@ -3283,8 +3288,8 @@
   S.stage_j = stj;
   S.stage_k = stk;
   S.blk_cnt = bcnt;
-  S.gap_count = ctl + N_SEG;
-  S.overflow = ctl + N_SEG + 1;
+  S.gap_count = ctl + SEL_CTL_GAPS;
+  S.overflow = ctl + SEL_CTL_OVERFLOW;
   return S;
 }
 
@@ -3428,7 +3433,7 @@
   NTS_WS(d_tcnt, uint32_t*, "sel_tile_cnt", n_kt * 4 + 8);
   NTS_WS(d_tord, uint8_t*, "sel_tile_ord", n_kt);
   NTS_WS(d_tscan, uint64_t*, "sel_tile_scan", n_kt * 8);
-  NTS_WS(d_ctl, unsigned long long*, "sel_ctl", (N_SEG + 2) * 8);
+  NTS_WS(d_ctl, unsigned long long*, "sel_ctl", SEL_CTL_WORDS * 8);
   const uint64_t gap_cap = V / w + g->n_rec + 16;
   NTS_WS(d_glo, uint64_t*, "gap_lo", gap_cap * 8);
   NTS_WS(d_ghi, uint64_t*, "gap_hi", gap_cap * 8);
@@ -3436,24 +3441,39 @@
                             : (uint64_t)((double)V * frac * std::min(1.0, 1.5 * plan.p + (accept_list ? 1e-4 : 0.02)) * 1.25 / N_SEG) + 8192;
   const bool elim_on = sel_hi && !(NTS_KNOB("NTS_SELECT_ELIM") && atoi(NTS_KNOB("NTS_SELECT_ELIM")) == 0);
   if (elim_on && !ctx->elim_needs_full_cap) cseg_cap = cseg_cap / 2 + 8192;
-  unsigned long long ctl[N_SEG + 1];
+  uint32_t tpw = (uint32_t)std::min<uint64_t>(16, std::max<uint64_t>(1, n_kt / (256ull * 32ull * 2ull)));
+  if (const char* e = NTS_KNOB("NTS_HI_TPW")) tpw = (uint32_t)std::max(1, std::min(64, atoi(e)));
+  const uint64_t n_waves = (n_kt + tpw - 1) / tpw;
+  NTS_WS(d_wcnt, uint32_t*, "sel_wave_cnt", (sel_hi ? n_waves : 1) * 4);
+  const bool win_direct_ok = sel_hi && !(NTS_KNOB("NTS_WIN_DIRECT") && atoi(NTS_KNOB("NTS_WIN_DIRECT")) == 0) && w <= SLOT_WALK * HIW_TILE;
+  uint32_t slot_G = 1, slot_S = 1;
+  if (win_direct_ok) {
+    const double per_wave = (double)tpw * HIW_TILE * std::min(1.0, (double)prune_c / (double)w) * (filter ? std::min(1.0, std::max(plan.p, 0.01)) : 1.0) * (elim_on ? 0.35 : 1.0);
+    slot_G = (uint32_t)std::min<double>(SLOT_G_MAX, std::max(1.0, std::floor((double)SPARSE_BLOCK / std::max(per_wave, 1.0) + 0.5)));
+    const double winners = (double)slot_G * tpw * HIW_TILE * 2.0 / (double)w;
+    const uint64_t most = ((uint64_t)slot_G * tpw * 64ull * hi_per + SPARSE_BLOCK - 1) / SPARSE_BLOCK;
+    slot_S = (uint32_t)std::min<uint64_t>(most, std::max<uint64_t>(1, (uint64_t)std::ceil(1.6 * winners / SPARSE_BLOCK)));
+  }
+  unsigned long long ctl[SEL_CTL_WORDS];
   std::vector<uint64_t> glo(GAP_PEEK), ghi(GAP_PEEK);
   uint64_t m = 0, n_gap = 0, n_sparse = 0;
   uint64_t *d_sj = nullptr, *d_sk = nullptr;
   for (int attempt = 0; attempt < 2; ++attempt) {
     const uint64_t m_max = cseg_cap * N_SEG;
-    const uint64_t n_blk = (m_max + SPARSE_BLOCK - 1) / SPARSE_BLOCK;
+    const bool direct = win_direct_ok && !ctx->win_direct_off;
+    const uint64_t n_slot_wg = (n_waves + slot_G - 1) / slot_G;
+    const uint64_t n_blk = direct ? n_slot_wg * slot_S : (m_max + SPARSE_BLOCK - 1) / SPARSE_BLOCK;
     const uint64_t slot_words = sel_hi ? n_kt * 64ull * hi_per : 0ull;
     d_sj = (uint64_t*)ws_get(ctx, "sel_seg_j", (slot_words + m_max) * 8);
     d_sk = (uint64_t*)ws_get(ctx, "sel_seg_key", (slot_words + m_max) * 8);
-    NTS_WS(d_pj, uint64_t*, "cand_j", m_max * 8);
-    NTS_WS(d_pk, uint64_t*, "cand_key", m_max * 8);
+    NTS_WS(d_pj, uint64_t*, "cand_j", (direct ? 1 : m_max) * 8);
+    NTS_WS(d_pk, uint64_t*, "cand_key", (direct ? 1 : m_max) * 8);
     NTS_WS(d_stj, uint64_t*, "stage_j", n_blk * SPARSE_BLOCK * 8);
     NTS_WS(d_stk, uint64_t*, "stage_k", n_blk * SPARSE_BLOCK * 8);
     NTS_WS(d_bcnt, uint64_t*, "blk_cnt", n_blk * 8);
     NTS_WS(d_bscan, uint64_t*, "blk_scan", n_blk * 8);
     if (!d_sj || !d_sk) return NTS_ENOMEM;
-    if (!ctx->sel_ctl_clean) HIP_TRY(ctx, hipMemsetAsync(d_ctl, 0, (N_SEG + 2) * 8, ctx->stream));
+    if (!ctx->sel_ctl_clean) HIP_TRY(ctx, hipMemsetAsync(d_ctl, 0, SEL_CTL_WORDS * 8, ctx->stream));
     ctx->sel_ctl_clean = false;
     if (!accept_list) {
       if (int rc_pk = ensure_pack(ctx, g)) return rc_pk;
@@ -3522,6 +3542,7 @@
       S.tile_cnt = d_tcnt;
       S.tile_ordered = d_tord;
       S.w_elim = (NTS_KNOB("NTS_SELECT_ELIM") && atoi(NTS_KNOB("NTS_SELECT_ELIM")) == 0) ? 0u : w;
+      S.wave_cnt = d_wcnt;
       const bool chained = g_live_contexts.load() > 1 && ctx->device < 32 && !(NTS_KNOB("NTS_SELECT_CHAIN") && atoi(NTS_KNOB("NTS_SELECT_CHAIN")) == 0);
       std::unique_lock<std::mutex> chain_lock(nts_chain::mu, std::defer_lock);
       if (chained) {
@@ -3548,9 +3569,6 @@
       }
       const uint32_t nch = (k + 3) / 4;
       if (sel_hi) {
-        const uint64_t waves_wanted = 256ull * 32ull * 2ull;
-        uint32_t tpw = (uint32_t)std::min<uint64_t>(16, std::max<uint64_t>(1, n_kt / waves_wanted));
-        if (const char* e = NTS_KNOB("NTS_HI_TPW")) tpw = (uint32_t)std::max(1, std::min(64, atoi(e)));
         const uint64_t per_wg = (uint64_t)HIW_WAVES * tpw;
         const dim3 grid((uint32_t)((n_kt + per_wg - 1) / per_wg));
         if (filter && hi_per == 2)
@@ -3567,7 +3585,7 @@
       else
         NTS_LAUNCH(k_hash_select<8>, dim3((uint32_t)n_kt), dim3(HASH_THREADS), 0, ctx->stream, S);
     }
-    {
+    if (!direct) {
       ScopedTimer t(ctx, "cand_compact");
       if (int rc_s = scan_counts<uint32_t>(ctx, d_tcnt, n_kt, d_tscan)) return rc_s;
       if (sel_hi)
@@ -3587,16 +3605,32 @@
     Q.no_gaps = every_window ? 1u : 0u;
     {
       ScopedTimer t(ctx, "sparse_win");
-      NTS_LAUNCH(k_sparse_win, dim3((uint32_t)n_blk), dim3(SPARSE_THREADS), 0, ctx->stream, Q);
+      if (direct) {
+        SlotParams D;
+        D.seg_j = d_sj;
+        D.seg_key = d_sk;
+        D.wave_cnt = d_wcnt;
+        D.tile_off = d_toff;
+        D.tile_cnt = d_tcnt;
+        D.n_tiles = n_kt;
+        D.n_waves = (uint32_t)n_waves;
+        D.region = tpw * 64u * hi_per;
+        D.G = slot_G;
+        D.S = slot_S;
+        D.ctl = d_ctl;
+        NTS_LAUNCH(k_sparse_win_slots, dim3((uint32_t)n_slot_wg), dim3(SPARSE_THREADS), 0, ctx->stream, Q, D);
+      } else {
+        NTS_LAUNCH(k_sparse_win, dim3((uint32_t)n_blk), dim3(SPARSE_THREADS), 0, ctx->stream, Q);
+      }
       if (int rc_s = scan_counts<uint64_t>(ctx, d_bcnt, n_blk, d_bscan)) return rc_s;
     }
     HIP_TRY(ctx, hipGetLastError());
     uint64_t last_scan = 0, last_cnt = 0, listed = 0;
     {
-      static_assert(N_SEG + 7 + 2 * GAP_PEEK < MAIL_WORDS - 8, "mailbox too small (the last word is the arrival flag)");
+      static_assert(SEL_CTL_WORDS + 6 + 2 * GAP_PEEK < MAIL_WORDS - 8, "mailbox too small (the last word is the arrival flag)");
       const uint32_t peek = (uint32_t)std::min<uint64_t>(GAP_PEEK, gap_cap);
       Mail mb(ctx);
-      const uint32_t a_ctl = mb.add(d_ctl, N_SEG + 1);
+      const uint32_t a_ctl = mb.add(d_ctl, SEL_CTL_WORDS);
       const uint32_t a_scan = mb.add(d_bscan + (n_blk - 1), 1);
       const uint32_t a_cnt = mb.add(d_bcnt + (n_blk - 1), 1);
       const uint32_t a_tscan = mb.add(d_tscan + (n_kt - 1), 1);
@@ -3612,10 +3646,10 @@
       }
       HIP_TRY(ctx, hipGetLastError());
       if ((rc_m = mb.wait(ctx))) return rc_m;
-      for (uint32_t i = 0; i <= N_SEG; ++i) ctl[i] = ctx->mail[a_ctl + i];
+      for (uint32_t i = 0; i < SEL_CTL_WORDS; ++i) ctl[i] = ctx->mail[a_ctl + i];
       last_scan = ctx->mail[a_scan];
       last_cnt = ctx->mail[a_cnt];
-      listed = ctx->mail[a_tscan] + (uint32_t)(ctx->mail[a_tcnt] >> (32 * ((n_kt - 1) & 1ull)));
+      listed = direct ? ctl[SEL_CTL_LISTED] : ctx->mail[a_tscan] + (uint32_t)(ctx->mail[a_tcnt] >> (32 * ((n_kt - 1) & 1ull)));
       memcpy(glo.data(), ctx->mail + a_lo, (size_t)peek * 8);
       memcpy(ghi.data(), ctx->mail + a_hi, (size_t)peek * 8);
       if (tiers) {
@@ -3623,6 +3657,13 @@
         ctx->last_tier_rounds = ctx->mail[a_tier + 1];
       }
     }
+    ctx->last_win_direct = direct && !ctl[SEL_CTL_GENERAL];
+    if (direct && ctl[SEL_CTL_GENERAL]) {
+      if (NTS_KNOB("NTS_DEBUG_RETRY")) fprintf(stderr, "[select] attempt %d: window decision on the slots gave up\n", attempt);
+      ctx->win_direct_off = true;
+      --attempt;
+      continue;
+    }
     uint64_t worst = 0;
     m = 0;
     for (uint32_t s = 0; s < N_SEG; ++s) {
@@ -3634,7 +3675,7 @@
     ctx->last_many_listed = sel_hi ? m : 0;
     if (sel_hi) {
       m = listed;
-      if (listed > m_max) worst = std::max<uint64_t>(worst, listed / N_SEG + 1);
+      if (!direct && listed > m_max) worst = std::max<uint64_t>(worst, listed / N_SEG + 1);
     }
     if (NTS_KNOB("NTS_DEBUG_RETRY")) fprintf(stderr, "[select] attempt %d: worst segment %llu of %llu, listed %llu, tiers %d\n", attempt, (unsigned long long)worst, (unsigned long long)cseg_cap, (unsigned long long)m, tiers ? 1 : 0);
     if (worst <= cseg_cap) break;
@@ -3879,6 +3920,14 @@
   return NTS_OK;
 }
 
+extern "C" int nts_win_direct_stats(nts_ctx* ctx, uint32_t* used_by_last_sketch, uint32_t* given_up)
+{
+  if (!ctx) return NTS_EINVAL;
+  if (used_by_last_sketch) *used_by_last_sketch = ctx->last_win_direct ? 1u : 0u;
+  if (given_up) *given_up = ctx->win_direct_off ? 1u : 0u;
+  return NTS_OK;
+}
+
 extern "C" int nts_sketch_stats(nts_ctx* ctx, uint64_t* candidates, uint64_t* uncovered_ranges, uint64_t* uncovered_kmers, uint32_t* prune_c_used)
 {
   if (!ctx) return NTS_EINVAL;
@@ -3975,17 +4024,17 @@
       }
       SK_HIP(hipGetLastError());
     }
-    uint64_t* const sel_ctl = plan.sel != SketchSel::Dense ? (uint64_t*)ws_get(ctx, "sel_ctl", (N_SEG + 2) * 8) : nullptr;
+    uint64_t* const sel_ctl = plan.sel != SketchSel::Dense ? (uint64_t*)ws_get(ctx, "sel_ctl", SEL_CTL_WORDS * 8) : nullptr;
     if (!res.d_ctl) {
       Mail done(ctx);
-      if (sel_ctl) done.clear_after(sel_ctl, N_SEG + 2);
+      if (sel_ctl) done.clear_after(sel_ctl, SEL_CTL_WORDS);
       SK_TRY(done.post(ctx));
       ctx->sel_ctl_clean = sel_ctl != nullptr;
       break;
     }
     Mail mb(ctx);
     const uint32_t at = mb.add(res.d_ctl, 3);
-    if (sel_ctl) mb.clear_after(sel_ctl, N_SEG + 2);
+    if (sel_ctl) mb.clear_after(sel_ctl, SEL_CTL_WORDS);
     SK_TRY(mb.post(ctx));
     ctx->sel_ctl_clean = sel_ctl != nullptr;
     if (ctx->mail[at + 2] == 0) {
diff --git a/ntsynt_amd/device.py b/ntsynt_amd/device.py
--- a/ntsynt_amd/device.py
+++ b/ntsynt_amd/device.py
@@ -156,7 +156,10 @@
     def path_stats(self):
         a, b, c = u64(), u64(), ctypes.c_uint32()
         self.check(self.lib.nts_path_stats(self.h, ctypes.byref(a), ctypes.byref(b), ctypes.byref(c)), "nts_path_stats")
-        return {"sketch_many_listed": a.value, "bf_direct_indices": b.value, "bf_list_fallback": c.value}
+        d, e = ctypes.c_uint32(), ctypes.c_uint32()
+        self.check(self.lib.nts_win_direct_stats(self.h, ctypes.byref(d), ctypes.byref(e)), "nts_win_direct_stats")
+        return {"sketch_many_listed": a.value, "bf_direct_indices": b.value, "bf_list_fallback": c.value,
+                "sketch_win_direct": bool(d.value), "sketch_win_direct_given_up": bool(e.value)}
 
     def bf_level_stats(self):
         a, b = ctypes.c_uint32(), u64()
```
